# nwihardjo/SpaghettiSearch

Hardware: AMD Instinct MI355X
Metric: pagerank_iters_per_sec (higher is better)
Workload: dtype f64

## Files before the change

spaghettisearch_amd/csrc/ctx.hip:

```cpp
#include "common.hpp"
#include <chrono>

#include <unordered_map>

namespace ss {

namespace {
struct Pool {
    std::mutex mu;
    std::multimap<std::pair<int, size_t>, void*> free_blocks;
    std::unordered_map<void*, std::pair<int, size_t>> live;
    size_t held = 0, limit = (size_t)64 << 30;
    double miss_ms = 0.0;
    uint64_t misses = 0;
    int contexts = 0;
};
Pool& pool() { static Pool* p = new Pool(); return *p; }
size_t size_class(size_t b) {
    if (b <= 4096) return 4096;
    size_t p2 = 4096;
    while (p2 < b) p2 <<= 1;
    if (p2 <= ((size_t)1 << 20)) return p2;
    const size_t step = p2 >> 4;
    return (b + step - 1) / step * step;
}
}

hipError_t pool_alloc(void** out, size_t bytes) {
    Pool& P = pool();
    const size_t cls = size_class(bytes);
    int dev = 0;
    (void)hipGetDevice(&dev);
    {
        std::lock_guard<std::mutex> lk(P.mu);
        auto it = P.free_blocks.find({dev, cls});
        if (it != P.free_blocks.end()) {
            *out = it->second;
            P.free_blocks.erase(it);
            P.held -= cls;
            P.live[*out] = {dev, cls};
            return hipSuccess;
        }
    }
    const auto tm0 = std::chrono::steady_clock::now();
    hipError_t e = hipMalloc(out, cls);
    {
        std::lock_guard<std::mutex> lk(P.mu);
        P.miss_ms += std::chrono::duration<double, std::milli>(std::chrono::steady_clock::now() - tm0).count();
        P.misses++;
    }
    if (e != hipSuccess) {
        (void)hipGetLastError();
        pool_trim();
        e = hipMalloc(out, cls);
    }
    if (e == hipSuccess) {
        std::lock_guard<std::mutex> lk(P.mu);
        P.live[*out] = {dev, cls};
    }
    return e;
}

static thread_local bool t_device_idle = false;

void pool_free_batch(void* const* blocks, size_t count) {
    if (!count) return;
    {
        int cur = 0;
        (void)hipGetDevice(&cur);
        if (device_wedged(cur)) return;
    }
    (void)hipDeviceSynchronize();
    t_device_idle = true;
    for (size_t i = 0; i < count; i++) pool_free(blocks[i]);
    t_device_idle = false;
}

void pool_free(void* p) {
    if (!p) return;
    Pool& P = pool();
    size_t cls = 0, limit = 0;
    int dev = 0;
    {
        std::lock_guard<std::mutex> lk(P.mu);
        auto it = P.live.find(p);
        if (it != P.live.end()) { dev = it->second.first; cls = it->second.second; P.live.erase(it); }
        limit = P.limit;
    }
    if (device_wedged(dev)) return;
    if (cls && cls <= limit / 2) {
        int cur = 0;
        (void)hipGetDevice(&cur);
        if (cur != dev || !t_device_idle) {
            if (cur != dev) (void)hipSetDevice(dev);
            (void)hipDeviceSynchronize();
            if (cur != dev) (void)hipSetDevice(cur);
        }
        std::vector<void*> evict;
        {
            std::lock_guard<std::mutex> lk(P.mu);
            while (P.held + cls > P.limit && !P.free_blocks.empty()) {
                auto last = std::prev(P.free_blocks.end());
                if (last->first.second <= cls) break;
                evict.push_back(last->second);
                P.held -= last->first.second;
                P.free_blocks.erase(last);
            }
            if (P.held + cls <= P.limit) {
                P.free_blocks.emplace(std::make_pair(dev, cls), p);
                P.held += cls;
                p = nullptr;
            }
        }
        for (void* q : evict) (void)hipFree(q);
        if (!p) return;
    }
    (void)hipFree(p);
}

void pool_stats(uint64_t* misses, double* miss_ms) {
    std::lock_guard<std::mutex> lk(pool().mu);
    *misses = pool().misses;
    *miss_ms = pool().miss_ms;
}
void pool_context_count(int delta) {
    bool last = false;
    {
        std::lock_guard<std::mutex> lk(pool().mu);
        pool().contexts += delta;
        last = delta < 0 && pool().contexts <= 0;
    }
    if (last) pool_trim();
}

void pool_trim() {
    Pool& P = pool();
    std::multimap<std::pair<int, size_t>, void*> take;
    {
        std::lock_guard<std::mutex> lk(P.mu);
        take.swap(P.free_blocks);
        P.held = 0;
    }
    for (auto& kv : take) (void)hipFree(kv.second);
}

void pool_set_limit(size_t bytes) {
    {
        std::lock_guard<std::mutex> lk(pool().mu);
        pool().limit = bytes;
    }
    pool_trim();
}

static std::mutex g_err_mu;
static std::string g_err;
void set_global_error(const std::string& msg) {
    std::lock_guard<std::mutex> lk(g_err_mu);
    g_err = msg;
}
}

extern "C" {

int32_t ss_abi_version(void) { return SS_ABI_VERSION; }

int32_t ss_init(int32_t device_id, ss_ctx** out) {
    if (!out) {
        ss::set_global_error("ss_init: out is NULL");
        return SS_ERR_INVALID;
    }
    *out = nullptr;
    int n_dev = 0;
    hipError_t e = hipGetDeviceCount(&n_dev);
    if (e != hipSuccess || n_dev <= 0) {
        ss::set_global_error(std::string("ss_init: no HIP device (") + hipGetErrorString(e) + ")");
        return SS_ERR_NO_DEVICE;
    }
    if (device_id < 0 || device_id >= n_dev) {
        ss::set_global_error("ss_init: device_id out of range");
        return SS_ERR_INVALID;
    }
    ss_ctx* ctx = new (std::nothrow) ss_ctx();
    if (!ctx) return SS_ERR_OOM;
    ctx->device = device_id;
    if ((e = hipSetDevice(device_id)) != hipSuccess) {
        ss::set_global_error(std::string("ss_init: hipSetDevice: ") + hipGetErrorString(e));
        delete ctx;
        return SS_ERR_NO_DEVICE;
    }
    hipDeviceProp_t prop;
    if ((e = hipGetDeviceProperties(&prop, device_id)) != hipSuccess) {
        ss::set_global_error(std::string("ss_init: hipGetDeviceProperties: ") + hipGetErrorString(e));
        delete ctx;
        return SS_ERR_NO_DEVICE;
    }
    if (std::strncmp(prop.gcnArchName, "gfx950", 6) != 0) {
        ss::set_global_error(std::string("ss_init: device is ") + prop.gcnArchName +
                             ", this library is built for gfx950 (MI355X) only");
        delete ctx;
        return SS_ERR_NO_DEVICE;
    }
    ctx->cu_count = prop.multiProcessorCount;
    ctx->total_mem = prop.totalGlobalMem;
    if ((e = hipStreamCreateWithFlags(&ctx->own_stream, hipStreamNonBlocking)) != hipSuccess) {
        ss::set_global_error(std::string("ss_init: hipStreamCreate: ") + hipGetErrorString(e));
        delete ctx;
        return SS_ERR_HIP;
    }
    ctx->stream = ctx->own_stream;
    int prio_lo = 0, prio_hi = 0;
    (void)hipDeviceGetStreamPriorityRange(&prio_lo, &prio_hi);
    if ((e = hipStreamCreateWithPriority(&ctx->comm_stream, hipStreamNonBlocking, prio_hi)) != hipSuccess) {
        ss::set_global_error(std::string("ss_init: hipStreamCreate (comm): ") + hipGetErrorString(e));
        (void)hipStreamDestroy(ctx->own_stream);
        delete ctx;
        return SS_ERR_HIP;
    }
    for (int k = 0; k < 3; k++)
        for (int j = 0; j < 2; j++)
            if ((e = hipEventCreate(&ctx->ev[k][j])) != hipSuccess) {
                ss::set_global_error(std::string("ss_init: hipEventCreate: ") + hipGetErrorString(e));
                delete ctx;
                return SS_ERR_HIP;
            }
    if ((e = hipHostMalloc(reinterpret_cast<void**>(&ctx->h_pin), ss_ctx::PIN_SCRATCH, hipHostMallocDefault)) != hipSuccess) {
        ss::set_global_error(std::string("ss_init: hipHostMalloc: ") + hipGetErrorString(e));
        delete ctx;
        return SS_ERR_HIP;
    }
    ss::pool_context_count(+1);
    *out = ctx;
    return SS_OK;
}

int32_t ss_shutdown(ss_ctx* ctx) {
    if (!ctx) return SS_ERR_INVALID;
    (void)hipSetDevice(ctx->device);
    const bool stuck = !ss::try_unwedge(ctx);
    (void)ss_comm_destroy(ctx);
    if (!stuck) (void)hipStreamSynchronize(ctx->stream);
    for (int k = 0; k < 3; k++)
        for (int j = 0; j < 2; j++)
            if (ctx->ev[k][j]) (void)hipEventDestroy(ctx->ev[k][j]);
    if (ctx->comm_stream && !stuck) { (void)hipStreamSynchronize(ctx->comm_stream); (void)hipStreamDestroy(ctx->comm_stream); }
    for (hipStream_t ws : ctx->wave_stream)
        if (ws && !stuck) { (void)hipStreamSynchronize(ws); (void)hipStreamDestroy(ws); }
    if (ctx->own_stream && !stuck) (void)hipStreamDestroy(ctx->own_stream);
    if (ctx->h_pin) (void)hipHostFree(ctx->h_pin);
    for (auto& b : ctx->pin_cache) (void)hipHostFree(b.p);
    delete ctx;
    ss::pool_context_count(-1);
    return SS_OK;
}

int32_t ss_set_stream(ss_ctx* ctx, void* hip_stream) {
    if (!ctx) return SS_ERR_INVALID;
    std::lock_guard<std::recursive_mutex> lk(ctx->mu);
    SS_HIP(ctx, hipStreamSynchronize(ctx->stream));
    ctx->stream = hip_stream ? reinterpret_cast<hipStream_t>(hip_stream) : ctx->own_stream;
    return SS_OK;
}

static const char* const k_option_names[] = {
    "comm.timeout_ms",
    "pr.force_narrow",
    "pr.wire_f32",
    "pr.narrow_wave",
    "pr.t_quad",
    "pr.blocks_per_cu",
    "mem.pool_mb",
    "pr.deal_snake",
    "pr.affine_lag",
    "pr.affine",
    "pr.items_per_wave",
    "pr.persistent",
    "pr.persistent_blocks",
    "pr.n_class_order",
    "pr.class_order",
    "pr.stagger",
    "pr.deal_global",
    "pr.share_zero_rows",
    "pr.item_turns",
    "graph.late_free",
    "pr.trace",
    "score.collect_pinned",
    "score.pipeline_slices",
    "score.timing",
    "score.trace",
    "pr.probe_hot",
    "pr.topic_blocks",
    "tfidf.blocks",
    "tfidf.bucket_shift",
    "tfidf.head_min_run",
    "tfidf.bucket_min",
    "score.wave",
    "score.wave_max_terms",
    "score.wave_min_list",
    "score.wave_share_pct",
    "score.wave_slice_target",
    "score.wave_big_pct",
    "score.wave_big_x100",
    "score.small",
    "score.small_max_batch",
    "score.small_batch",
    "score.small_cap",
    "score.pipeline",
    "score.grade_slices",
    "score.wave_small_x100",
    "score.exact_all",
    "score.slice_target",
    "score.separate_merge",
    "passage.lds_events",
    "lexicon.chunk_terms",
};

int32_t ss_set_option(ss_ctx* ctx, const char* name, int64_t value) {
    if (!ctx || !name) return SS_ERR_INVALID;
    std::lock_guard<std::recursive_mutex> lk(ctx->mu);
    for (const char* n : k_option_names)
        if (std::strcmp(n, name) == 0) {
            if (value == SS_OPTION_DEFAULT) ctx->options.erase(name);
            else ctx->options[name] = value;
            if (std::strcmp(name, "mem.pool_mb") == 0) ss::pool_set_limit(value == SS_OPTION_DEFAULT ? (size_t)64 << 30 : (size_t)std::max<int64_t>(0, value) << 20);
            return SS_OK;
        }
    return ctx->fail(SS_ERR_INVALID, "ss_set_option: unknown option '%s'", name);
}

int32_t ss_synchronize(ss_ctx* ctx) {
    if (!ctx) return SS_ERR_INVALID;
    std::lock_guard<std::recursive_mutex> lk(ctx->mu);
    SS_HIP(ctx, hipSetDevice(ctx->device));
    SS_TRY(ss::sync_bounded(ctx, ctx->stream, "ss_synchronize"));
    return SS_OK;
}

const char* ss_last_error(ss_ctx* ctx) {
    if (ctx) return ctx->last_error.c_str();
    static thread_local std::string tl;
    {
        std::lock_guard<std::mutex> lk(ss::g_err_mu);
        tl = ss::g_err;
    }
    return tl.c_str();
}

int32_t ss_last_kernel_ms(ss_ctx* ctx, int32_t kind, float* ms_out) {
    if (!ctx || !ms_out || kind < 0 || kind > 2) return SS_ERR_INVALID;
    std::lock_guard<std::recursive_mutex> lk(ctx->mu);
    if (!ctx->ev_valid[kind]) return ctx->fail(SS_ERR_STATE, "ss_last_kernel_ms: no timed call of kind %d yet", kind);
    SS_HIP(ctx, hipEventSynchronize(ctx->ev[kind][1]));
    SS_HIP(ctx, hipEventElapsedTime(ms_out, ctx->ev[kind][0], ctx->ev[kind][1]));
    return SS_OK;
}

}
```

spaghettisearch_amd/csrc/pagerank.hip:

```cpp
#include "pr_device.hpp"

#include <algorithm>
#include <chrono>
#include <cmath>
#include <memory>

namespace {

__global__ void k_pr_item_ranges(WorkItem* __restrict__ work, uint32_t n_items, const uint32_t* __restrict__ in_ptr) {
    const uint32_t i = blockIdx.x * blockDim.x + threadIdx.x;
    if (i >= n_items) return;
    WorkItem w = work[i];
    switch (w.kind) {
        case V_ROWW: w.beg = in_ptr[w.row]; w.end = in_ptr[w.row + 1]; break;
        case V_SEG:
            w.beg = in_ptr[w.row] + w.count * SEGW;
            w.end = min(in_ptr[w.row + 1], w.beg + SEGW);
            break;
        case V_QUAD:
        case V_DEG: w.beg = in_ptr[w.row]; w.end = in_ptr[w.row + w.count]; break;
        default: return;
    }
    work[i] = w;
}

__global__ __launch_bounds__(TPB) void k_pr_remap_src(const uint32_t* __restrict__ in_src, uint32_t* __restrict__ out, size_t n_edges, uint32_t pos_nd,
                                                      uint32_t cnt_nd, const uint32_t* __restrict__ outdeg, const uint32_t* __restrict__ sh_deg,
                                                      uint32_t n_shared, uint32_t zrow) {
    for (size_t e = (size_t)blockIdx.x * TPB + threadIdx.x; e < n_edges; e += (size_t)gridDim.x * TPB) {
        uint32_t w = NT_LOAD(&in_src[e]);
        const uint32_t s = w & SRC_MASK;
        if (s >= pos_nd) {
            uint32_t row = zrow;
            if (s < cnt_nd && n_shared) {
                const uint32_t od = outdeg[s];
                uint32_t lo = 0, hi = n_shared;
                while (lo < hi) {
                    const uint32_t mid = (lo + hi) >> 1;
                    if (sh_deg[mid] < od) lo = mid + 1; else hi = mid;
                }
                if (lo < n_shared && sh_deg[lo] == od) row = zrow + 1 + lo;
            }
            w = (w & ~SRC_MASK) | row;
        }
        NT_STORE(w, &out[e]);
    }
}

template <int GW>
__global__ __launch_bounds__(TPB) void k_pr_begin(PrParams p) {
    const int lane = threadIdx.x & 63;
    const int t = lane % GW;
    const double x0 = p.x0[t];
    double* __restrict__ Tw = p.tab_wr[1];
    double csum = 0.0;
    for (uint32_t i = blockIdx.x * TPB + threadIdx.x; i < p.n_shared * (uint32_t)GW; i += gridDim.x * TPB)
        Tw[(size_t)(p.zrow + 1) * GW + i] = p.d * x0 / (double)p.sh_deg[i / GW];
    const size_t n_el = ((size_t)p.sl_nd + p.sl_d) * GW;
    for (size_t i = (size_t)blockIdx.x * TPB + threadIdx.x; i < n_el; i += (size_t)gridDim.x * TPB) {
        const uint32_t lrow = (uint32_t)(i / GW);
        const bool real = lrow < p.sl_nd ? lrow < p.cnt_nd : (lrow - p.sl_nd) < p.cnt_d;
        p.x[i] = real ? x0 : 0.0;
        if (lrow < p.sl_nd) {
            double c = 0.0;
            if (real) c = p.d * x0 / (double)p.outdeg[lrow];
            if ((p.world == 1 || lrow + 2 < p.sl_nd) && lrow < p.tab_rows) Tw[i] = c;
            csum += c;
        }
    }
    block_reduce_and_publish<GW>(p, 0.0, csum, Tw, true);
}

template <int GW>
__global__ void k_pr_finalize(PrParams p, const double* __restrict__ table, int is_begin) {
    if (threadIdx.x != 0 || blockIdx.x != 0) return;
    if (!is_begin && p.ctl->n_active == 0) return;
    double dl[MAXK], cs[MAXK];
    for (int k = 0; k < MAXK; k++) { dl[k] = 0.0; cs[k] = 0.0; }
    for (int r = 0; r < p.world; r++) {
        const size_t base = ((size_t)r * p.sl_nd + (p.sl_nd - 2)) * GW;
        for (int k = 0; k < GW; k++) {
            cs[k] += table[base + k];
            dl[k] += table[base + GW + k];
        }
    }
    finalize_ctl(p, dl, cs, is_begin != 0);
}

template <int GW>
__global__ void k_pr_read(const double* __restrict__ x, const PrCtl* __restrict__ ctl, const uint32_t* __restrict__ old_id,
                          uint32_t sl_nd, uint32_t cnt_nd, uint32_t pos_nd, uint32_t sl_d, uint32_t cnt_d, uint32_t pos_d,
                          uint64_t id0_nd, uint64_t id0_d, int k_topics, uint64_t out_stride,
                          int by_original_id, uint32_t* __restrict__ ids_out, double* __restrict__ out,
                          const uint32_t* __restrict__ memb, uint32_t ts_mask) {
    const size_t n_rows = (size_t)cnt_nd + cnt_d;
    size_t i = (size_t)blockIdx.x * blockDim.x + threadIdx.x;
    if (i >= n_rows) return;
    const uint32_t lrow = i < cnt_nd ? (uint32_t)i : sl_nd + (uint32_t)(i - cnt_nd);
    const uint64_t iid = lrow < sl_nd ? id0_nd + lrow : id0_d + (lrow - sl_nd);
    const uint32_t orig = old_id[iid];
    const size_t o = by_original_id ? (size_t)orig : i;
    if (ids_out) ids_out[i] = orig;
    const bool zero = lrow < sl_nd ? lrow >= pos_nd : (lrow - sl_nd) >= pos_d;
    const uint32_t mb = memb ? memb[lrow] & ts_mask : 0u;
    for (int k = 0; k < k_topics; k++)
        out[(size_t)k * out_stride + o] = zero ? (((mb >> k) & 1u) ? ctl->xz_in[k] : ctl->xz[k]) : x[(size_t)lrow * GW + k];
}

__global__ void k_pr_memb(const uint64_t* __restrict__ set_ptr, const uint32_t* __restrict__ set_nodes, int k_topics, uint64_t n_nodes,
                          const uint32_t* __restrict__ new_id, uint64_t nd_int, uint32_t sl_nd, uint32_t sl_d, int rank,
                          uint32_t* __restrict__ memb, uint32_t* __restrict__ seen, uint32_t* __restrict__ err) {
    const uint64_t total = set_ptr[k_topics];
    for (uint64_t i = (uint64_t)blockIdx.x * blockDim.x + threadIdx.x; i < total; i += (uint64_t)gridDim.x * blockDim.x) {
        int k = 0;
        while (k + 1 < k_topics && set_ptr[k + 1] <= i) k++;
        const uint32_t v = set_nodes[i];
        if ((uint64_t)v >= n_nodes) { atomicOr(err, 1u); continue; }
        if (atomicOr(&seen[v], 1u << k) & (1u << k)) { atomicOr(err, 2u); continue; }
        const uint64_t iid = new_id[v];
        uint32_t lrow;
        int owner;
        if (iid < nd_int) { owner = (int)(iid / sl_nd); lrow = (uint32_t)(iid % sl_nd); }
        else { owner = (int)((iid - nd_int) / sl_d); lrow = sl_nd + (uint32_t)((iid - nd_int) % sl_d); }
        if (owner == rank) atomicOr(&memb[lrow], 1u << k);
    }
}
__global__ void k_pr_memb_zero_count(const uint32_t* __restrict__ memb, uint32_t sl_nd, uint32_t cnt_nd, uint32_t pos_nd, uint32_t cnt_d,
                                     uint32_t pos_d, int k_topics, unsigned long long* __restrict__ cnt) {
    const uint32_t z_nd = cnt_nd - pos_nd, n_zero = z_nd + (cnt_d - pos_d);
    for (uint32_t i = blockIdx.x * blockDim.x + threadIdx.x; i < n_zero; i += gridDim.x * blockDim.x) {
        const uint32_t lrow = i < z_nd ? pos_nd + i : sl_nd + pos_d + (i - z_nd);
        const uint32_t mb = memb[lrow];
        for (int k = 0; k < k_topics; k++)
            if ((mb >> k) & 1u) atomicAdd(&cnt[k], 1ull);
    }
}

template <int GW, int POL>
__global__ __launch_bounds__(TPB) void k_pr_probe(const double* __restrict__ T, const uint32_t* __restrict__ in_src, size_t n_edges,
                                                  uint32_t n_rows, int mode, double* __restrict__ sink, uint32_t hot) {
    if constexpr (GW >= 8) {
        constexpr int NSLOT = 64 / GW;
        const int lane = threadIdx.x & 63, wave = threadIdx.x >> 6;
        const int t = lane % GW, slot = lane / GW, gbase = lane - t;
        const size_t groups = (size_t)gridDim.x * WAVES * NSLOT;
        const size_t gi = ((size_t)blockIdx.x * WAVES + wave) * NSLOT + slot;
        const size_t n_chunks = n_edges / CH;
        const size_t per = (n_chunks + groups - 1) / groups;
        size_t c = min(gi * per, n_chunks);
        const size_t c_hi = min(c + per, n_chunks);
        double acc = 0.0;
        for (; c < c_hi; c++) {
            constexpr int R = CH / GW;
            uint32_t src[R];
#pragma unroll
            for (int r = 0; r < R; r++) {
                const size_t e = c * CH + (size_t)(r * GW + t);
                uint32_t v = NT_LOAD(&in_src[e]) & SRC_MASK;
                if (mode == 1) v = (uint32_t)(((uint64_t)(v * 2654435761u + (uint32_t)e * 40503u) * n_rows) >> 32);
                if (mode == 2) v = (uint32_t)(e % n_rows);
                src[r] = v;
            }
            double v[CH];
#pragma unroll
            for (int j = 0; j < CH; j++) {
                const uint32_t sj = (uint32_t)__shfl((int)src[j / GW], gbase + (j % GW), 64);
                const double* a = &T[(size_t)sj * GW + t];
                if constexpr (POL == 0) v[j] = *a;
                else if constexpr (POL == 1) v[j] = __builtin_nontemporal_load(a);
                else if constexpr (POL == 2) v[j] = __hip_atomic_load(a, __ATOMIC_RELAXED, __HIP_MEMORY_SCOPE_AGENT);
                else if constexpr (POL == 3) v[j] = sj < hot ? *a : __builtin_nontemporal_load(a);
                else v[j] = sj < hot ? *a : __hip_atomic_load(a, __ATOMIC_RELAXED, __HIP_MEMORY_SCOPE_AGENT);
            }
#pragma unroll
            for (int j = 0; j < CH; j++) acc += v[j];
        }
        sink[((size_t)blockIdx.x * TPB + threadIdx.x)] = acc;
    }
}

}

namespace {

void pick_kernel(const ss_ctx* ctx, ss_pr* pr, int k, uint64_t table_rows) {
    const bool force_narrow = ctx->opt("pr.force_narrow", 0) != 0, narrow_wave = ctx->opt("pr.narrow_wave", 1) != 0;
    if (k > 2) {
        pr->kernel = PR_SWEEP;
        pr->gw = k <= 8 ? 8 : 16;
    } else if (force_narrow) {
        pr->kernel = PR_STEP;
        pr->gw = k;
    } else if (narrow_wave) {
        pr->kernel = PR_SWEEP_N;
        pr->gw = k;
    } else if (table_rows * 64 <= (64ull << 20)) {
        pr->kernel = PR_SWEEP;
        pr->gw = 8;
    } else {
        pr->kernel = PR_STEP;
        pr->gw = k;
    }
    pr->nwave = pr->kernel == PR_SWEEP_N;
    const int64_t want = ctx->opt("pr.persistent", 0);
    pr->persist_mode = want == 2 ? 2 : 1;
    pr->persist = pr->nwave && pr->g->world == 1 && !ctx->opt("pr.affine", 0) && want > 0;
}

template <int GW>
void launch_begin(ss_pr* pr, hipStream_t st, unsigned nb) {
    hipLaunchKernelGGL(k_pr_begin<GW>, dim3(nb), dim3(TPB), 0, st, pr->prm);
}
template <int GW>
void launch_finalize(ss_pr* pr, hipStream_t st, int is_begin) {
    hipLaunchKernelGGL(k_pr_finalize<GW>, dim3(1), dim3(64), 0, st, pr->prm, (const double*)pr->tab0.p, is_begin);
}
template <int GW>
__global__ __launch_bounds__(TPB) void k_pr_read_orig(const double* __restrict__ x, const PrCtl* __restrict__ ctl, const uint32_t* __restrict__ new_id,
                                                      uint64_t n, uint32_t sl_nd, uint32_t pos_nd, uint32_t pos_d, int k_topics,
                                                      double* __restrict__ out, const uint32_t* __restrict__ memb, uint32_t ts_mask) {
    const uint64_t v = (uint64_t)blockIdx.x * blockDim.x + threadIdx.x;
    if (v >= n) return;
    const uint32_t lrow = new_id[v];
    const bool zero = lrow < sl_nd ? lrow >= pos_nd : (lrow - sl_nd) >= pos_d;
    double r[GW];
    if (!zero) {
        if constexpr (GW >= 2) {
            const double2* const row = reinterpret_cast<const double2*>(x + (size_t)lrow * GW);
#pragma unroll
            for (int j = 0; j < GW / 2; j++) { const double2 t = row[j]; r[2 * j] = t.x; r[2 * j + 1] = t.y; }
        } else {
            r[0] = x[lrow];
        }
    } else {
        const uint32_t mb = memb ? memb[lrow] & ts_mask : 0u;
#pragma unroll
        for (int k = 0; k < GW; k++) r[k] = ((mb >> k) & 1u) ? ctl->xz_in[k] : ctl->xz[k];
    }
#pragma unroll
    for (int k = 0; k < GW; k++)
        if (k < k_topics) out[(size_t)k * n + v] = r[k];
}

template <int GW>
void launch_read(ss_pr* pr, hipStream_t st, int by_orig, uint64_t stride, uint32_t* ids, double* out) {
    const ss_graph* g = pr->g;
    const size_t n_rows = (size_t)g->cnt_nd + g->cnt_d;
    if (!n_rows) return;
    if (by_orig && g->world == 1 && !ids && stride == g->n) {
        hipLaunchKernelGGL(k_pr_read_orig<GW>, dim3(ss::div_up(g->n, TPB)), dim3(TPB), 0, st, (const double*)pr->x.p, (const PrCtl*)pr->ctl.p,
                           (const uint32_t*)g->new_id.p, g->n, g->sl_nd, pr->prm.pos_nd, pr->prm.pos_d, pr->k, out, pr->prm.memb, pr->prm.ts_mask);
        return;
    }
    hipLaunchKernelGGL(k_pr_read<GW>, dim3(ss::div_up(n_rows, TPB)), dim3(TPB), 0, st, (const double*)pr->x.p,
                       (const PrCtl*)pr->ctl.p, (const uint32_t*)g->old_id.p, g->sl_nd, g->cnt_nd, pr->prm.pos_nd, g->sl_d, g->cnt_d,
                       pr->prm.pos_d,
                       (uint64_t)g->rank * g->sl_nd, g->nd_int + (uint64_t)g->rank * g->sl_d, pr->k, stride, by_orig, ids, out,
                       pr->prm.memb, pr->prm.ts_mask);
}

#define SS_GW_DISPATCH(gw, fn, ...)          \
    switch (gw) {                            \
        case 1: fn<1>(__VA_ARGS__); break;   \
        case 2: fn<2>(__VA_ARGS__); break;   \
        case 8: fn<8>(__VA_ARGS__); break;   \
        default: fn<16>(__VA_ARGS__); break; \
    }

}

namespace ss {
unsigned begin_blocks(const ss_pr* pr) { return std::max(1u, std::min(2048u, ss::div_up((size_t)pr->g->n_local() * pr->gw, TPB))); }
void pr_launch_begin(ss_pr* pr, hipStream_t st, unsigned nb) { SS_GW_DISPATCH(pr->gw, launch_begin, pr, st, nb); }
void pr_launch_step(ss_pr* pr, hipStream_t st) {
    switch (pr->kernel) {
        case PR_STEP: pr_step_launch(pr, st); break;
        case PR_SWEEP: pr_sweep_launch(pr, st); break;
        case PR_SWEEP_N: pr_sweep_n_launch(pr, st); break;
    }
}
void pr_launch_finalize(ss_pr* pr, hipStream_t st, int is_begin) { SS_GW_DISPATCH(pr->gw, launch_finalize, pr, st, is_begin); }
}

namespace {

PlanOptions plan_options(const ss_ctx* ctx, const ss_pr* pr, size_t n_local) {
    const bool small = n_local <= ((size_t)4 << 20);
    PlanOptions o;
    o.t_quad = (uint32_t)ctx->opt("pr.t_quad", pr->nwave ? 256 : 128);
    o.item_turns = (uint32_t)std::max<int64_t>(1, std::min<int64_t>(64, ctx->opt("pr.item_turns", pr->nwave ? (small ? 1 : 4) : (small ? 4 : 8))));
    o.items_per_wave = pr->nwave ? (size_t)std::max<int64_t>(1, ctx->opt("pr.items_per_wave", 4)) : 1;
    o.deal_snake = ctx->opt("pr.deal_snake", PlanOptions::AUTO);
    o.deal_global = ctx->opt("pr.deal_global", pr->nwave && pr->gw == 1 ? 1 : 2);
    o.blocks_per_cu = ctx->opt("pr.blocks_per_cu", PlanOptions::AUTO);
    o.class_order = ctx->opt("pr.class_order", 235401);
    o.n_class_order = ctx->opt("pr.n_class_order", small ? 2310 : 123);
    o.stagger = ctx->opt("pr.stagger", 0);
    return o;
}

constexpr int OCC_MULTI_N = 3;
int blocks_per_cu(int row, int gw) {
    static std::mutex occ_mu;
    static int occ_cache[4][MAXK + 1] = {};
    std::lock_guard<std::mutex> lk_occ(occ_mu);
    int& occ = occ_cache[row][gw];
    if (!occ) {
        int per_cu = 0;
        switch (row) {
            case PR_STEP: per_cu = ss::pr_step_occupancy(gw); break;
            case PR_SWEEP: per_cu = ss::pr_sweep_occupancy(gw); break;
            case PR_SWEEP_N: per_cu = ss::pr_sweep_n_occupancy(gw); break;
            default: per_cu = ss::pr_multi_n_occupancy(gw); break;
        }
        occ = std::max(per_cu, 1);
    }
    return occ;
}
unsigned grid_for(const ss_ctx* ctx, const ss_pr* pr, const PlanOptions& opt, int per_cu, size_t n_items) {
    per_cu = (int)std::max<int64_t>(1, opt.blocks_per_cu == PlanOptions::AUTO ? per_cu : opt.blocks_per_cu);
    if (pr->persist) {
        const int admit = std::max(1, blocks_per_cu(OCC_MULTI_N, pr->gw) - 2);
        per_cu = (int)std::max<int64_t>(1, std::min<int64_t>(std::min(admit, std::max(1, per_cu / 2)), ctx->opt("pr.persistent_blocks", 4)));
    }
    return pr->kernel != PR_STEP ? (unsigned)std::min<size_t>(std::max<size_t>(1, ss::div_up(n_items, (size_t)WAVES * opt.items_per_wave)), (size_t)ctx->cu_count * per_cu)
                                 : (unsigned)std::min<size_t>(n_items, (size_t)ctx->cu_count * 8);
}

void fill_params(ss_pr* pr, const Cut& cut, const PlanOptions& opt, double damping, double eps, int32_t max_iter, int32_t k_topics) {
    const ss_graph* g = pr->g;
    PrParams& p = pr->prm;
    p.in_ptr = g->in_ptr.p;
    p.in_src = g->in_src.p;
    p.outdeg = g->outdeg.p;
    p.x = pr->x.p;
    if (g->world == 1) {
        p.tab_rd[0] = pr->tab0.p; p.tab_wr[0] = pr->tab1.p;
        p.tab_rd[1] = pr->tab1.p; p.tab_wr[1] = pr->tab0.p;
    } else {
        p.tab_rd[0] = p.tab_rd[1] = pr->tab0.p;
        p.tab_wr[0] = p.tab_wr[1] = pr->send.p;
    }
    p.work = pr->work.p;
    p.partials = pr->partials.p;
    p.segpart = pr->segpart.p;
    p.rowticket = pr->rowticket.p;
    p.ctl = pr->ctl.p;
    p.x0 = pr->x0.p;
    p.d = damping;
    p.teleport = 1.0 - damping;
    p.eps = eps;
    p.tele_n = p.teleport * (double)g->n;
    p.max_iter = max_iter;
    p.k_topics = k_topics;
    p.world = g->world;
    p.sl_nd = g->sl_nd;
    p.cnt_nd = g->cnt_nd;
    p.sl_d = g->sl_d;
    p.cnt_d = g->cnt_d;
    p.seg_edges = cut.seg_edges;
    p.n_items = (uint32_t)cut.items.size();
    p.pos_nd = cut.pos_nd;
    p.pos_d = cut.pos_d;
    p.zrow = (uint32_t)g->nd_int;
    p.tab_rows = g->sl_nd;
    p.woff = pr->woff.p;
    p.stagger_div = opt.stagger != 0 ? (uint32_t)std::max(g->ctx->cu_count, 1) : 0u;
    p.stagger_code = opt.stagger >= 10 ? (uint32_t)(opt.stagger - 10) : 0u;
    p.class_order = pack_class_order(opt.class_order);
    p.n_order = pack_n_order(opt.n_class_order);
}

uint64_t fnv1a(const void* q, size_t n, uint64_t h = 0xcbf29ce484222325ull) {
    const unsigned char* b = static_cast<const unsigned char*>(q);
    for (size_t i = 0; i < n; i++) { h ^= b[i]; h *= 0x100000001b3ull; }
    return h;
}
void trace_plan(const ss_pr* pr, const std::vector<WorkItem>& work, const std::vector<uint32_t>& woff) {
    const PrParams& p = pr->prm;
    const double sd[] = {p.d, p.teleport, p.eps, p.tele_n};
    const uint32_t su[] = {(uint32_t)p.max_iter, (uint32_t)p.k_topics, (uint32_t)p.world, p.sl_nd, p.cnt_nd, p.sl_d, p.cnt_d, p.seg_edges, p.n_items,
                           p.pos_nd, p.pos_d, p.ts_mask, p.zrow, p.stagger_div, p.stagger_code, p.class_order, p.n_order};
    fprintf(stderr, "[pr trace] plan: work %016llx (%zu items)  woff %016llx  params %016llx  nblocks %u\n",
            (unsigned long long)fnv1a(work.data(), work.size() * sizeof(WorkItem)), work.size(),
            (unsigned long long)fnv1a(woff.data(), woff.size() * sizeof(uint32_t)),
            (unsigned long long)fnv1a(su, sizeof(su), fnv1a(sd, sizeof(sd))), pr->nblocks);
}

int32_t alloc_tables(ss_pr* pr, hipStream_t st, size_t rows) {
    const ss_graph* g = pr->g;
    ss_ctx* ctx = g->ctx;
    const size_t GW = (size_t)pr->gw;
    SS_HIP(ctx, pr->tab0.alloc(rows * GW));
    SS_HIP(ctx, hipMemsetAsync(pr->tab0.p, 0, std::max<size_t>(pr->tab0.bytes(), 8), st));
    if (g->world == 1) {
        SS_HIP(ctx, pr->tab1.alloc(rows * GW));
        SS_HIP(ctx, hipMemsetAsync(pr->tab1.p, 0, std::max<size_t>(pr->tab1.bytes(), 8), st));
    } else {
        SS_HIP(ctx, pr->send.alloc((size_t)g->sl_nd * GW));
        SS_HIP(ctx, hipMemsetAsync(pr->send.p, 0, std::max<size_t>(pr->send.bytes(), 8), st));
    }
    return SS_OK;
}
int32_t unshare_rows(ss_pr* pr, hipStream_t st) {
    if (!pr->prm.share) return SS_OK;
    const ss_graph* g = pr->g;
    SS_HIP(g->ctx, hipStreamSynchronize(st));
    SS_TRY(alloc_tables(pr, st, (size_t)g->nd_int + 1));
    pr->src_shared.release();
    pr->sh_deg.release();
    PrParams& p = pr->prm;
    p.tab_rd[0] = pr->tab0.p; p.tab_wr[0] = pr->tab1.p;
    p.tab_rd[1] = pr->tab1.p; p.tab_wr[1] = pr->tab0.p;
    p.in_src = g->in_src.p;
    p.sh_deg = nullptr;
    p.n_shared = 0;
    p.share = 0;
    p.zrow = (uint32_t)g->nd_int;
    p.tab_rows = g->sl_nd;
    return SS_OK;
}

#ifdef SS_PR_WAVETIME
void dump_wave_loads(const Cut& cut, const std::vector<double>& cost, const std::vector<uint32_t>& owner, uint32_t nw) {
    FILE* f = open_dump("pr_load.csv");
    if (!f) return;
    std::vector<double> wl(nw, 0.0), wcls((size_t)nw * 6, 0.0);
    for (size_t i = 0; i < cut.items.size(); i++) {
        int kc = 0; while (kc < 5 && i >= cut.vbeg[kc + 1]) kc++;
        wl[owner[i]] += cost[i]; wcls[(size_t)owner[i] * 6 + kc] += cost[i];
    }
    fprintf(f, "wave,load,c0,c1,c2,c3,c4,c5\n");
    for (uint32_t w = 0; w < nw; w++) fprintf(f, "%u,%.2f,%.2f,%.2f,%.2f,%.2f,%.2f,%.2f\n", w, wl[w], wcls[(size_t)w * 6], wcls[(size_t)w * 6 + 1], wcls[(size_t)w * 6 + 2], wcls[(size_t)w * 6 + 3], wcls[(size_t)w * 6 + 4], wcls[(size_t)w * 6 + 5]);
    fclose(f);
}
#endif

}

extern "C" {

int32_t ss_pr_create(ss_graph* g, double damping, double eps, int32_t max_iter, int32_t k_topics,
                     const int32_t* n_topic, ss_pr** out) {
    if (!g) return SS_ERR_INVALID;
    ss_ctx* ctx = g->ctx;
    std::lock_guard<std::recursive_mutex> lk(ctx->mu);
    if (!out) return ctx->fail(SS_ERR_INVALID, "ss_pr_create: out is NULL");
    *out = nullptr;
    if (k_topics < 1 || !n_topic) return ctx->fail(SS_ERR_INVALID, "ss_pr_create: k_topics < 1 or n_topic NULL");
    if (k_topics > MAXK) return ctx->fail(SS_ERR_UNSUPPORTED, "ss_pr_create: k_topics %d > %d per state (ss_pagerank_run splits larger K)", k_topics, MAXK);
    SS_HIP(ctx, hipSetDevice(ctx->device));
    hipStream_t st = ctx->stream;

    ss_pr* pr = new (std::nothrow) ss_pr();
    if (!pr) return ctx->fail(SS_ERR_OOM, "ss_pr_create: host OOM");
    std::unique_ptr<ss_pr> guard(pr);
    pr->g = g;
    pr->k = k_topics;
    pick_kernel(ctx, pr, k_topics, g->nd_int);
    const int GW = pr->gw;
    const bool vitems = pr->kernel != PR_STEP;
    const int GI = pr->nwave ? 8 : GW;
    const size_t n_local = g->n_local();
    if (((uint64_t)g->nd_int + 1) * GW * 8 >= (1ull << 32))
        return ctx->fail(SS_ERR_UNSUPPORTED, "ss_pr_create: contribution table of %llu rows x %d topics exceeds 4 GiB (shard the graph over more ranks)",
                         (unsigned long long)g->nd_int, GW);

    const bool trace = ctx->opt("pr.trace", 0) != 0;
    auto t_now = [] { return std::chrono::steady_clock::now(); };
    auto t_ms = [](std::chrono::steady_clock::time_point a, std::chrono::steady_clock::time_point b) { return std::chrono::duration<double, std::milli>(b - a).count(); };
    SS_HIP(ctx, pr->x.alloc(n_local * GW));
    bool share = GW >= 8 && g->world == 1 && ctx->opt("pr.affine", 0) == 0 && ctx->opt("pr.share_zero_rows", 1) != 0;
    if (!share) SS_TRY(alloc_tables(pr, st, (size_t)g->nd_int + 1));

    const auto tc0 = t_now();
    const PlanOptions opt = plan_options(ctx, pr, n_local);
    Cut cut = cut_items(g->h_indeg_nd, g->h_indeg_d, g->sl_nd, GI, pr->nwave, opt);
    const uint32_t n_tail = g->cnt_nd - cut.pos_nd;
    struct PinGuard { ss_ctx* c; void* p = nullptr; size_t cap = 0; ~PinGuard() { c->pin_free(p, cap); } } tail_od{ctx};
    if (share && n_tail == 0) {
        share = false;
        SS_TRY(alloc_tables(pr, st, (size_t)g->nd_int + 1));
    }
    if (share) {
        tail_od.p = ctx->pin_alloc((size_t)n_tail * sizeof(uint32_t), &tail_od.cap);
        if (!tail_od.p) return ctx->fail(SS_ERR_OOM, "ss_pr_create: no pinned host memory for %u out-degrees", n_tail);
        SS_HIP(ctx, hipMemcpyAsync(tail_od.p, g->outdeg.p + cut.pos_nd, (size_t)n_tail * sizeof(uint32_t), hipMemcpyDeviceToHost, st));
    }
    const auto tc1 = t_now();
    const int per_cu = blocks_per_cu(pr->kernel, GW);
    const auto tc1a = t_now();
    pr->nblocks = grid_for(ctx, pr, opt, per_cu, cut.items.size());
    static const std::vector<uint32_t> no_woff;
    const std::vector<uint32_t>* woff = &no_woff;
    if (vitems) {
        const uint32_t nw = pr->nblocks * WAVES;
        const auto td0 = t_now();
        const std::vector<double>& cost = item_costs(cut, g->h_indeg_nd, g->h_indeg_d, g->sl_nd, GI, pr->nwave);
        const auto td0a = t_now();
        std::vector<uint32_t>& owner = deal_items(cut, cost, nw, pr->nwave, opt);
#ifdef SS_PR_WAVETIME
        dump_wave_loads(cut, cost, owner, nw);
#endif
        const auto td1 = t_now();
        if (trace) fprintf(stderr, "[pr trace]   deal: occupancy query %.2f ms, costs %.3f ms, owners %.3f ms\n", t_ms(tc1, tc1a), t_ms(td0, td0a), t_ms(td0a, td1));
        woff = &place_items(cut, owner, nw);
        if (trace) fprintf(stderr, "[pr trace]   deal: placement %.3f ms\n", t_ms(td1, t_now()));
    }
    const std::vector<WorkItem>& items = cut.items;

    g->settle();
    const auto tc2 = t_now();
    SharedRows sh;
    if (share) {
        SS_HIP(ctx, hipStreamSynchronize(st));
        const auto ts0 = t_now();
        sh = plan_shared_rows(static_cast<const uint32_t*>(tail_od.p), n_tail, cut.pos_nd);
        const auto ts1 = t_now();
        SS_TRY(alloc_tables(pr, st, (size_t)sh.table_rows));
        SS_HIP(ctx, pr->sh_deg.alloc(sh.deg.size()));
        SS_HIP(ctx, hipMemcpyAsync(pr->sh_deg.p, sh.deg.data(), sh.deg.size() * sizeof(uint32_t), hipMemcpyHostToDevice, st));
        SS_HIP(ctx, pr->src_shared.alloc(g->e_local));
        if (g->e_local)
            hipLaunchKernelGGL(k_pr_remap_src, dim3((unsigned)std::min<uint64_t>(ss::div_up(g->e_local, TPB), (uint64_t)ctx->cu_count * 16)), dim3(TPB), 0, st,
                               (const uint32_t*)g->in_src.p, pr->src_shared.p, (size_t)g->e_local, cut.pos_nd, g->cnt_nd, (const uint32_t*)g->outdeg.p,
                               (const uint32_t*)pr->sh_deg.p, (uint32_t)sh.deg.size(), sh.zrow);
        if (trace) fprintf(stderr, "[pr trace]   shared rows: %u rows without in-edges -> %zu shared rows (host %.3f ms), table %llu rows\n", n_tail, sh.deg.size(),
                           t_ms(ts0, ts1), (unsigned long long)sh.table_rows);
    }
    SS_HIP(ctx, pr->partials.alloc(((size_t)std::max(pr->nblocks, ss::begin_blocks(pr)) + 8) * 2 * GW));
    SS_HIP(ctx, pr->segpart.alloc((size_t)std::max(cut.nsegs, 1u) * GW));
    SS_HIP(ctx, pr->rowticket.alloc(std::max(cut.nmulti, 1u)));
    SS_HIP(ctx, hipMemsetAsync(pr->rowticket.p, 0, pr->rowticket.bytes(), st));
    SS_HIP(ctx, pr->woff.alloc(std::max<size_t>(woff->size(), 8)));
    if (!woff->empty()) SS_HIP(ctx, hipMemcpyAsync(pr->woff.p, woff->data(), woff->size() * sizeof(uint32_t), hipMemcpyHostToDevice, st));
    SS_HIP(ctx, pr->work.alloc(items.size()));
    SS_HIP(ctx, hipMemcpyAsync(pr->work.p, items.data(), items.size() * sizeof(WorkItem), hipMemcpyHostToDevice, st));
    if (vitems)
        hipLaunchKernelGGL(k_pr_item_ranges, dim3(ss::div_up(items.size(), TPB)), dim3(TPB), 0, st, pr->work.p, (uint32_t)items.size(), (const uint32_t*)g->in_ptr.p);
    SS_HIP(ctx, pr->ctl.alloc(1));
    SS_HIP(ctx, hipMemsetAsync(pr->ctl.p, 0, sizeof(PrCtl), st));
    double h_x0[MAXK];
    for (int k = 0; k < MAXK; k++) h_x0[k] = k < k_topics ? 1.0 / (double)n_topic[k] : 0.0;
    SS_HIP(ctx, pr->x0.alloc(MAXK));
    SS_HIP(ctx, hipMemcpyAsync(pr->x0.p, h_x0, sizeof(h_x0), hipMemcpyHostToDevice, st));
    SS_HIP(ctx, hipStreamSynchronize(st));
    if (trace) fprintf(stderr, "[pr trace] ss_pr_create: build_work %.2f ms (%zu items), edge ranges + deal %.2f ms, alloc + upload %.2f ms\n", t_ms(tc0, tc1), items.size(), t_ms(tc1, tc2), t_ms(tc2, t_now()));
    if (trace) fprintf(stderr, "[pr trace] where the state lives: x %p  tab0 %p  tab1 %p  in_src %p  in_ptr %p  outdeg %p  work %p  woff %p\n", (void*)pr->x.p, (void*)pr->tab0.p,
                       (void*)pr->tab1.p, (void*)g->in_src.p, (void*)g->in_ptr.p, (void*)g->outdeg.p, (void*)pr->work.p, (void*)pr->woff.p);

    fill_params(pr, cut, opt, damping, eps, max_iter, k_topics);
    if (share) {
        PrParams& p = pr->prm;
        p.in_src = pr->src_shared.p;
        p.sh_deg = pr->sh_deg.p;
        p.n_shared = (uint32_t)sh.deg.size();
        p.share = 1;
        p.zrow = sh.zrow;
        p.tab_rows = cut.pos_nd;
    }
    if (trace) trace_plan(pr, items, *woff);
    g->users++;
    *out = guard.release();
    return SS_OK;
}

int32_t ss_pr_set_teleport(ss_pr* pr, const uint64_t* set_ptr, const uint32_t* set_nodes) {
    if (!pr) return SS_ERR_INVALID;
    ss_ctx* ctx = pr->g->ctx;
    std::lock_guard<std::recursive_mutex> lk(ctx->mu);
    SS_HIP(ctx, hipSetDevice(ctx->device));
    if (pr->begun) return ctx->fail(SS_ERR_STATE, "ss_pr_set_teleport: call before ss_pr_begin");
    hipStream_t st = ctx->stream;
    PrParams& p = pr->prm;
    if (!set_ptr) {
        p.memb = nullptr; p.tin = nullptr; p.nz_in = nullptr; p.ts_mask = 0;
        return SS_OK;
    }
    const ss_graph* g = pr->g;
    const int K = pr->k;
    SS_TRY(unshare_rows(pr, st));
    std::vector<uint64_t> h_ptr(K + 1);
    SS_HIP(ctx, ss::copy_in(ctx->stream, h_ptr.data(), set_ptr, (K + 1) * sizeof(uint64_t)));
    if (h_ptr[0] != 0) return ctx->fail(SS_ERR_INVALID, "ss_pr_set_teleport: set_ptr[0] != 0");
    for (int k = 0; k < K; k++)
        if (h_ptr[k + 1] < h_ptr[k]) return ctx->fail(SS_ERR_INVALID, "ss_pr_set_teleport: set_ptr not non-decreasing");
    const uint64_t total = h_ptr[K];
    if (total && !set_nodes) return ctx->fail(SS_ERR_INVALID, "ss_pr_set_teleport: set_nodes is NULL");
    double h_tin[MAXK];
    uint32_t mask = 0;
    for (int k = 0; k < MAXK; k++) {
        h_tin[k] = 0.0;
        if (k < K && h_ptr[k + 1] > h_ptr[k]) {
            mask |= 1u << k;
            h_tin[k] = p.teleport * (double)g->n / (double)(h_ptr[k + 1] - h_ptr[k]);
        }
    }
    const size_t n_local = g->n_local();
    ss::DevBuf<uint64_t> d_ptr;
    ss::DevBuf<uint32_t> d_nodes, d_err, d_seen;
    ss::DevBuf<unsigned long long> d_cnt;
    SS_HIP(ctx, d_ptr.alloc(K + 1));
    SS_HIP(ctx, d_seen.alloc(g->n));
    SS_HIP(ctx, hipMemsetAsync(d_seen.p, 0, std::max<size_t>(d_seen.bytes(), 4), st));
    SS_HIP(ctx, d_nodes.alloc(total));
    SS_HIP(ctx, d_err.alloc(1));
    SS_HIP(ctx, d_cnt.alloc(MAXK));
    SS_HIP(ctx, pr->memb.alloc(n_local));
    SS_HIP(ctx, pr->tin.alloc(MAXK));
    SS_HIP(ctx, pr->nz_in.alloc(MAXK));
    SS_HIP(ctx, hipMemcpyAsync(d_ptr.p, h_ptr.data(), (K + 1) * sizeof(uint64_t), hipMemcpyHostToDevice, st));
    if (total) SS_HIP(ctx, hipMemcpyAsync(d_nodes.p, set_nodes, total * sizeof(uint32_t), hipMemcpyDefault, st));
    SS_HIP(ctx, hipMemsetAsync(pr->memb.p, 0, std::max<size_t>(pr->memb.bytes(), 4), st));
    SS_HIP(ctx, hipMemsetAsync(d_err.p, 0, sizeof(uint32_t), st));
    SS_HIP(ctx, hipMemsetAsync(d_cnt.p, 0, MAXK * sizeof(unsigned long long), st));
    if (total)
        hipLaunchKernelGGL(k_pr_memb, dim3(std::min<unsigned>(ss::div_up(total, TPB), 4096u)), dim3(TPB), 0, st, (const uint64_t*)d_ptr.p,
                           (const uint32_t*)d_nodes.p, K, g->n, (const uint32_t*)g->new_id.p, g->nd_int, std::max(g->sl_nd, 1u), std::max(g->sl_d, 1u),
                           g->rank, pr->memb.p, d_seen.p, d_err.p);
    const uint32_t n_zero = (g->cnt_nd - p.pos_nd) + (g->cnt_d - p.pos_d);
    if (n_zero)
        hipLaunchKernelGGL(k_pr_memb_zero_count, dim3(std::min<unsigned>(ss::div_up(n_zero, TPB), 4096u)), dim3(TPB), 0, st,
                           (const uint32_t*)pr->memb.p, g->sl_nd, g->cnt_nd, p.pos_nd, g->cnt_d, p.pos_d, K, d_cnt.p);
    SS_HIP(ctx, hipGetLastError());
    uint32_t h_err = 0;
    unsigned long long h_cnt[MAXK];
    SS_HIP(ctx, ss::fetch(ctx, st, &h_err, d_err.p, sizeof(h_err), h_cnt, d_cnt.p, sizeof(h_cnt)));
    if (h_err & 1u) return ctx->fail(SS_ERR_INVALID, "ss_pr_set_teleport: a teleport set holds a node id >= n_nodes");
    if (h_err & 2u) return ctx->fail(SS_ERR_INVALID, "ss_pr_set_teleport: a teleport set lists a node twice (the ids of a set must be distinct)");
    double h_nz[MAXK];
    for (int k = 0; k < MAXK; k++) h_nz[k] = (double)h_cnt[k];
    SS_HIP(ctx, hipMemcpyAsync(pr->tin.p, h_tin, sizeof(h_tin), hipMemcpyHostToDevice, st));
    SS_HIP(ctx, hipMemcpyAsync(pr->nz_in.p, h_nz, sizeof(h_nz), hipMemcpyHostToDevice, st));
    SS_HIP(ctx, hipStreamSynchronize(st));
    p.memb = pr->memb.p;
    p.tin = pr->tin.p;
    p.nz_in = pr->nz_in.p;
    p.ts_mask = mask;
    return SS_OK;
}

int32_t ss_pr_destroy(ss_pr* pr) {
#ifdef SS_PR_WAVETIME
    if (pr) ss::pr_dump_wave_times(pr);
#endif

    if (!pr) return SS_ERR_INVALID;
    ss_ctx* ctx = pr->g->ctx;
    std::lock_guard<std::recursive_mutex> lk(ctx->mu);
    (void)hipSetDevice(ctx->device);
    if (!ss::device_wedged(ctx->device)) {
        (void)hipStreamSynchronize(ctx->stream);
        (void)hipStreamSynchronize(ctx->comm_stream);
    }
    pr->g->users--;
    delete pr;
    return SS_OK;
}

int32_t ss_pr_begin(ss_pr* pr) {
    if (!pr) return SS_ERR_INVALID;
    ss_ctx* ctx = pr->g->ctx;
    std::lock_guard<std::recursive_mutex> lk(ctx->mu);
    SS_HIP(ctx, hipSetDevice(ctx->device));
    if (pr->need_finalize) return ctx->fail(SS_ERR_STATE, "ss_pr_begin: pending exchange/finalize");
    SS_HIP(ctx, hipMemsetAsync(&pr->ctl.p->ticket, 0, sizeof(uint32_t), ctx->stream));
    ss::pr_launch_begin(pr, ctx->stream, ss::begin_blocks(pr));
    SS_HIP(ctx, hipGetLastError());
    pr->begun = true;
    if (pr->g->world > 1) {
        pr->need_finalize = true;
        pr->finalize_is_begin = true;
    }
    return SS_OK;
}

int32_t ss_pr_step(ss_pr* pr, int32_t n_steps) {
    if (!pr) return SS_ERR_INVALID;
    ss_ctx* ctx = pr->g->ctx;
    std::lock_guard<std::recursive_mutex> lk(ctx->mu);
    SS_HIP(ctx, hipSetDevice(ctx->device));
    if (!pr->begun) return ctx->fail(SS_ERR_STATE, "ss_pr_step: ss_pr_begin not called");
    if (pr->need_finalize) return ctx->fail(SS_ERR_STATE, "ss_pr_step: pending exchange/finalize");
    if (n_steps < 1) return ctx->fail(SS_ERR_INVALID, "ss_pr_step: n_steps < 1");
    if (pr->g->world > 1 && n_steps != 1) return ctx->fail(SS_ERR_INVALID, "ss_pr_step: world>1 needs an exchange after every step");
    SS_HIP(ctx, hipEventRecord(ctx->ev[0][0], ctx->stream));
    if (pr->persist && !pr->prm.memb && !pr->prm.aff) {
        ss::pr_multi_n_launch(pr, ctx->stream, (int)n_steps);
    } else {
        for (int i = 0; i < n_steps; i++) ss::pr_launch_step(pr, ctx->stream);
    }
    SS_HIP(ctx, hipEventRecord(ctx->ev[0][1], ctx->stream));
    ctx->ev_valid[0] = true;
    SS_HIP(ctx, hipGetLastError());
    if (pr->g->world > 1) {
        pr->need_finalize = true;
        pr->finalize_is_begin = false;
    }
    return SS_OK;
}

int32_t ss_pr_finalize(ss_pr* pr) {
    if (!pr) return SS_ERR_INVALID;
    ss_ctx* ctx = pr->g->ctx;
    std::lock_guard<std::recursive_mutex> lk(ctx->mu);
    SS_HIP(ctx, hipSetDevice(ctx->device));
    if (pr->g->world == 1) return ctx->fail(SS_ERR_STATE, "ss_pr_finalize: world==1 folds the finalize into the sweep");
    if (!pr->need_finalize) return ctx->fail(SS_ERR_STATE, "ss_pr_finalize: nothing to finalize");
    ss::pr_launch_finalize(pr, ctx->stream, pr->finalize_is_begin ? 1 : 0);
    SS_HIP(ctx, hipGetLastError());
    pr->need_finalize = false;
    return SS_OK;
}

int32_t ss_pr_exchange_buffers(ss_pr* pr, void** send_dev, uint64_t* send_bytes, void** recv_dev, uint64_t* recv_bytes) {
    if (!pr) return SS_ERR_INVALID;
    ss_ctx* ctx = pr->g->ctx;
    if (pr->g->world == 1) return ctx->fail(SS_ERR_STATE, "ss_pr_exchange_buffers: world==1 has no exchange");
    if (send_dev) *send_dev = pr->send.p;
    if (send_bytes) *send_bytes = pr->send.bytes();
    if (recv_dev) *recv_dev = pr->tab0.p;
    if (recv_bytes) *recv_bytes = (uint64_t)pr->g->nd_int * pr->gw * sizeof(double);
    return SS_OK;
}

int32_t ss_pr_exchange(ss_pr* pr, int32_t allreduce) {
    if (!pr) return SS_ERR_INVALID;
    ss_ctx* ctx = pr->g->ctx;
    std::lock_guard<std::recursive_mutex> lk(ctx->mu);
    SS_HIP(ctx, hipSetDevice(ctx->device));
    const ss_graph* g = pr->g;
    if (g->world == 1) return ctx->fail(SS_ERR_STATE, "ss_pr_exchange: world==1 has no exchange");
    if (!pr->need_finalize) return ctx->fail(SS_ERR_STATE, "ss_pr_exchange: nothing to exchange (call after ss_pr_begin / ss_pr_step)");
    if (!ctx->comm || ctx->comm_world != g->world || ctx->comm_rank != g->rank)
        return ctx->fail(SS_ERR_STATE, "ss_pr_exchange: the context's communicator (rank %d of %d) does not match the graph's shard (rank %d of %d)",
                         ctx->comm ? ctx->comm_rank : -1, ctx->comm ? ctx->comm_world : 0, g->rank, g->world);
    const size_t slice = (size_t)g->sl_nd * pr->gw;
    if (!allreduce && ctx->opt("pr.wire_f32", 0) != 0) {
        SS_HIP(ctx, ss::pr_wire_alloc(pr));
        ss::pr_wire_pack(pr, ctx->stream);
        SS_TRY(ss::comm_allgather(ctx, pr->wire_send.p, pr->wire_recv.p, ss::pr_wire_floats(pr) * sizeof(float)));
        ss::pr_wire_unpack(pr, ctx->stream);
        return SS_OK;
    }
    if (!allreduce) return ss::comm_allgather(ctx, pr->send.p, pr->tab0.p, slice * sizeof(double));
    SS_HIP(ctx, hipMemsetAsync(pr->tab0.p, 0, pr->tab0.bytes(), ctx->stream));
    SS_HIP(ctx, hipMemcpyAsync(pr->tab0.p + (size_t)g->rank * slice, pr->send.p, slice * sizeof(double), hipMemcpyDeviceToDevice, ctx->stream));
    return ss::comm_allreduce_f64(ctx, pr->tab0.p, pr->tab0.p, slice * (size_t)g->world);
}

int32_t ss_pr_status(ss_pr* pr, int32_t* iters_out, int32_t* n_active, int32_t* sweeps, double* last_delta_out,
                     double* last_total_out) {
    if (!pr) return SS_ERR_INVALID;
    ss_ctx* ctx = pr->g->ctx;
    std::lock_guard<std::recursive_mutex> lk(ctx->mu);
    SS_HIP(ctx, hipSetDevice(ctx->device));
    const PrCtl* hp = nullptr;
    SS_TRY(read_ctl(ctx, pr, ctx->stream, "ss_pr_status", &hp));
    const PrCtl h = *hp;
    if (h.stuck) return ctx->fail(SS_ERR_STATE, "ss_pr_status: the multi-sweep kernel gave up waiting between two sweeps (its grid of %u blocks was not resident: "
                                  "other kernels held the CUs for seconds); the state is void — set option pr.persistent = 0 and run again", pr->nblocks);
    for (int k = 0; k < pr->k; k++) {
        if (iters_out) iters_out[k] = h.iters[k];
        if (last_delta_out) last_delta_out[k] = h.delta[k];
        if (last_total_out) last_total_out[k] = h.S[k];
    }
    if (n_active) *n_active = h.n_active;
    if (sweeps) *sweeps = h.sweep;
    return SS_OK;
}

int32_t ss_pr_read_local(ss_pr* pr, uint32_t* ids_out, double* rank_out) {
    if (!pr || !rank_out) return SS_ERR_INVALID;
    ss_ctx* ctx = pr->g->ctx;
    std::lock_guard<std::recursive_mutex> lk(ctx->mu);
    SS_HIP(ctx, hipSetDevice(ctx->device));
    const ss_graph* g = pr->g;
    const size_t n_rows = (size_t)g->cnt_nd + g->cnt_d;
    ss::DevBuf<uint32_t> d_ids;
    ss::DevBuf<double> d_out;
    SS_HIP(ctx, d_ids.alloc(n_rows));
    SS_HIP(ctx, d_out.alloc(n_rows * pr->k));
    SS_GW_DISPATCH(pr->gw, launch_read, pr, ctx->stream, 0, (uint64_t)n_rows, d_ids.p, d_out.p);
    SS_HIP(ctx, hipGetLastError());
    if (ids_out && n_rows) SS_HIP(ctx, hipMemcpyAsync(ids_out, d_ids.p, n_rows * sizeof(uint32_t), hipMemcpyDefault, ctx->stream));
    if (n_rows) SS_HIP(ctx, hipMemcpyAsync(rank_out, d_out.p, n_rows * pr->k * sizeof(double), hipMemcpyDefault, ctx->stream));
    SS_HIP(ctx, hipStreamSynchronize(ctx->stream));
    return SS_OK;
}

int32_t ss_pr_read(ss_pr* pr, double* rank_out) {
    if (!pr || !rank_out) return SS_ERR_INVALID;
    ss_ctx* ctx = pr->g->ctx;
    std::lock_guard<std::recursive_mutex> lk(ctx->mu);
    SS_HIP(ctx, hipSetDevice(ctx->device));
    const ss_graph* g = pr->g;
    if (g->world != 1) return ctx->fail(SS_ERR_STATE, "ss_pr_read: world>1, use ss_pr_read_local");
    hipPointerAttribute_t pa{};
    const bool dev_out = hipPointerGetAttributes(&pa, rank_out) == hipSuccess && pa.type == hipMemoryTypeDevice;
    (void)hipGetLastError();
    ss::DevBuf<double> d_out;
    if (!dev_out) SS_HIP(ctx, d_out.alloc((size_t)g->n * pr->k));
    SS_GW_DISPATCH(pr->gw, launch_read, pr, ctx->stream, 1, (uint64_t)g->n, (uint32_t*)nullptr, dev_out ? rank_out : d_out.p);
    SS_HIP(ctx, hipGetLastError());
    if (!dev_out) SS_HIP(ctx, hipMemcpyAsync(rank_out, d_out.p, (size_t)g->n * pr->k * sizeof(double), hipMemcpyDefault, ctx->stream));
    SS_HIP(ctx, hipStreamSynchronize(ctx->stream));
    return SS_OK;
}

int32_t ss_pr_probe(ss_pr* pr, int32_t mode, int32_t n_reps, float* ms_out) {
    if (!pr || !ms_out) return SS_ERR_INVALID;
    ss_ctx* ctx = pr->g->ctx;
    std::lock_guard<std::recursive_mutex> lk(ctx->mu);
    SS_HIP(ctx, hipSetDevice(ctx->device));
    if (pr->gw < 8) return ctx->fail(SS_ERR_UNSUPPORTED, "ss_pr_probe: the probe mirrors the chunked gather of the K >= 5 kernels");
    if (mode < 0 || (mode & 7) > 2 || (mode >> 3) > 4 || n_reps < 1) return ctx->fail(SS_ERR_INVALID, "ss_pr_probe: mode 0..2 (+ 8 * gather cache policy 0..4), n_reps >= 1");
    const int pol = mode >> 3;
    mode &= 7;
    const uint32_t hot = (uint32_t)ctx->opt("pr.probe_hot", 24576);
    const ss_graph* g = pr->g;
    const unsigned nb = (unsigned)ctx->cu_count * 8;
    ss::DevBuf<double> sink;
    SS_HIP(ctx, sink.alloc((size_t)nb * TPB));
    hipEvent_t e0, e1;
    SS_HIP(ctx, hipEventCreate(&e0));
    SS_HIP(ctx, hipEventCreate(&e1));
    hipStream_t st = ctx->stream;
    ss::DevBuf<double> full;
    if (pr->prm.share) {
        SS_HIP(ctx, full.alloc(((size_t)g->nd_int + 1) * pr->gw));
        SS_HIP(ctx, hipMemsetAsync(full.p, 0, full.bytes(), ctx->stream));
    }
    const double* T = pr->prm.share ? full.p : pr->tab0.p;
    for (int r = 0; r < n_reps + 1; r++) {
        if (r == 1) SS_HIP(ctx, hipEventRecord(e0, st));
#define SS_PROBE_LAUNCH(GWV, POLV) hipLaunchKernelGGL((k_pr_probe<GWV, POLV>), dim3(nb), dim3(TPB), 0, st, T, (const uint32_t*)g->in_src.p, (size_t)g->e_local, (uint32_t)g->nd_int, mode, sink.p, hot)
        if (pr->gw == 8) SS_PROBE_LAUNCH(8, 0);
        else switch (pol) {
            case 0: SS_PROBE_LAUNCH(16, 0); break;
            case 1: SS_PROBE_LAUNCH(16, 1); break;
            case 2: SS_PROBE_LAUNCH(16, 2); break;
            case 3: SS_PROBE_LAUNCH(16, 3); break;
            default: SS_PROBE_LAUNCH(16, 4); break;
        }
    }
    SS_HIP(ctx, hipEventRecord(e1, st));
    SS_HIP(ctx, hipEventSynchronize(e1));
    float ms = 0.f;
    SS_HIP(ctx, hipEventElapsedTime(&ms, e0, e1));
    (void)hipEventDestroy(e0);
    (void)hipEventDestroy(e1);
    SS_HIP(ctx, hipGetLastError());
    *ms_out = ms / (float)n_reps;
    return SS_OK;
}

}
```

spaghettisearch_amd/csrc/pr_plan.hpp:

```cpp
#pragma once
#include "sorted_degrees.hpp"

#include <algorithm>
#include <cstdint>
#include <utility>
#include <vector>

namespace {

constexpr int TPB = 256;
constexpr int WAVES = TPB / 64;
constexpr int CH = 16;
constexpr uint32_t SEGW = 2048;

enum : uint32_t { W_SEG = 0, W_WAVE = 1, W_GROUP = 2, W_ZERO = 3,
                  V_SEG = 8,
                  V_ROWW = 9,
                  V_QUAD = 10,
                  V_DEG = 11,
                  V_ZERO = 12 };

struct WorkItem {
    uint32_t kind;
    uint32_t row;
    uint32_t count;
    uint32_t nseg;
    uint32_t sbase;
    uint32_t tix;
    uint32_t beg, end;
};

constexpr uint32_t plan_div_up(uint64_t a, uint64_t b) { return (uint32_t)((a + b - 1) / b); }

struct PlanOptions {
    static constexpr int64_t AUTO = INT64_MIN;
    uint32_t t_quad = 128;
    uint32_t item_turns = 4;
    size_t items_per_wave = 1;
    int64_t deal_snake = AUTO;
    int64_t deal_global = 2;
    int64_t blocks_per_cu = AUTO;
    int64_t class_order = 235401;
    int64_t n_class_order = 2310;
    int64_t stagger = 0;
};

struct PlanScratch {
    std::vector<WorkItem> seg, rwg, wav, grp, zer;
    std::vector<WorkItem> vseg, vroww, vquad, vdeg[3], vzero;
    std::vector<WorkItem> items, dealt;
    std::vector<double> cost, load;
    std::vector<uint32_t> owner, by_load, idx, order, bucket, woff, cnt;
    std::vector<std::pair<double, uint32_t>> key;
};
inline PlanScratch& plan_scratch() {
    static thread_local PlanScratch s;
    return s;
}

struct Cut {
    std::vector<WorkItem>& items;
    uint32_t nsegs = 0, nmulti = 0;
    uint32_t seg_edges = 0;
    uint32_t pos_nd = 0, pos_d = 0;
    uint32_t vbeg[7] = {0};
};

inline Cut cut_items(const ss::SortedDegrees& nd, const ss::SortedDegrees& d, uint32_t sl_nd, int gw, bool lane_rows, const PlanOptions& opt) {
    PlanScratch& s = plan_scratch();
    Cut cut{s.items};
    uint32_t& nsegs = cut.nsegs;
    uint32_t& nmulti = cut.nmulti;
    const uint32_t NSLOT = 64 / gw;
    const uint32_t T_SEG = 32 * NSLOT;
    const uint32_t T_WAVE = 2 * NSLOT;
    const uint32_t seg_edges = cut.seg_edges = 128 * NSLOT;
    auto &seg = s.seg, &rwg = s.rwg, &wav = s.wav, &grp = s.grp, &zer = s.zer;
    auto &vseg = s.vseg, &vroww = s.vroww, &vquad = s.vquad, &vzero = s.vzero;
    auto& vdeg = s.vdeg;
    for (auto* v : {&seg, &rwg, &wav, &grp, &zer, &vseg, &vroww, &vquad, &vdeg[0], &vdeg[1], &vdeg[2], &vzero}) v->clear();
    auto emit_v = [&](const ss::SortedDegrees& deg, uint32_t row0, bool non_dangling, uint32_t& n_pos) {
        const uint32_t cnt = (uint32_t)deg.size();
        const uint32_t T_MULTI = 4096, T_DEG = 8;
        const uint32_t T_QUAD = opt.t_quad;
        const uint32_t item_turns = opt.item_turns;
        size_t j_at = 0, j_lim = 0;
        const size_t n_run = deg.val.size();
        auto deg_at = [&](uint32_t r) -> uint32_t {
            while (deg.start[j_at + 1] <= r) j_at++;
            return deg.val[j_at];
        };
        auto end_above = [&](uint32_t lim) -> uint32_t {
            while (j_lim < n_run && deg.val[j_lim] > lim) j_lim++;
            return deg.start[j_lim];
        };
        uint32_t r = 0;
        for (; r < cnt && deg_at(r) > T_MULTI; r++) {
            const uint32_t ns = (deg_at(r) + SEGW - 1) / SEGW;
            const uint32_t tix = nmulti++;
            for (uint32_t sg = 0; sg < ns; sg++) vseg.push_back({V_SEG, row0 + r, sg, ns, nsegs, tix});
            nsegs += ns;
        }
        {
            const uint32_t end = std::min(cnt, end_above(T_QUAD));
            for (; r < end; r++) vroww.push_back({V_ROWW, row0 + r, 0, 0, 0, 0});
        }
        while (r < cnt && deg_at(r) > T_DEG) {
            const uint32_t nch = (deg_at(r) + CH - 1) / CH;
            const uint32_t max_groups = std::min<uint32_t>((uint32_t)gw, std::max<uint32_t>(1u, 2u * item_turns / nch));
            const uint32_t lim = std::max<uint32_t>(T_DEG, (nch - 1) * CH);
            const uint32_t end = end_above(lim);
            const uint32_t same = end > r ? end - r : 0u;
            const uint32_t rows = std::min<uint32_t>(same, max_groups * NSLOT);
            vquad.push_back({V_QUAD, row0 + r, rows, nch, 0, 0});
            r += rows;
        }
        while (r < cnt && deg_at(r) > 0) {
            const uint32_t D = deg_at(r);
            const uint32_t run = deg.start[j_at + 1] - r;
            const uint32_t R = D <= 2 ? 8 : D <= 4 ? 4 : 2;
            const uint32_t per_item = lane_rows ? 64u * item_turns : NSLOT * R * item_turns;
            auto& out = vdeg[R == 2 ? 0 : R == 4 ? 1 : 2];
            for (uint32_t o = 0; o < run; o += per_item) out.push_back({V_DEG, row0 + r + o, std::min(per_item, run - o), D, 0, 0});
            r += run;
        }
        n_pos = r;
        const uint32_t ZERO_ROWS = 16 * NSLOT;
        if (non_dangling)
            for (uint32_t o = r; o < cnt; o += ZERO_ROWS) vzero.push_back({V_ZERO, row0 + o, std::min<uint32_t>(ZERO_ROWS, cnt - o), 0, 0, 0});
    };
    auto emit = [&](const ss::SortedDegrees& deg, uint32_t row0, bool non_dangling, uint32_t& n_pos) {
        if (gw >= 8) { emit_v(deg, row0, non_dangling, n_pos); return; }
        const uint32_t cnt = (uint32_t)deg.size();
        const uint32_t a = deg.first_at_most(T_SEG);
        const uint32_t c = std::max(a, deg.first_at_most(0));
        for (uint32_t r = 0; r < a; r++) {
            const uint32_t ns = (deg[r] + seg_edges - 1) / seg_edges;
            const uint32_t tix = ns > 1 ? nmulti++ : 0;
            for (uint32_t sg = 0; sg < ns; sg++) seg.push_back({W_SEG, row0 + r, sg, ns, nsegs, tix});
            nsegs += ns;
        }
        {
            const uint32_t b = std::min(c, std::max(a, deg.first_at_most(T_WAVE)));
            for (uint32_t r = a; r < b; r += WAVES) wav.push_back({W_WAVE, row0 + r, std::min<uint32_t>(WAVES, b - r), 0, 0, 0});
            const uint32_t GROUP_ROWS = WAVES * NSLOT * 4;
            for (uint32_t r = b; r < c; r += GROUP_ROWS) grp.push_back({W_GROUP, row0 + r, std::min<uint32_t>(GROUP_ROWS, c - r), 0, 0, 0});
        }
        n_pos = c;
        const uint32_t ZERO_ROWS = (TPB * 8) / gw;
        if (non_dangling)
            for (uint32_t r = c; r < cnt; r += ZERO_ROWS) zer.push_back({W_ZERO, row0 + r, std::min<uint32_t>(ZERO_ROWS, cnt - r), 0, 0, 0});
    };
    emit(nd, 0, true, cut.pos_nd);
    const size_t vquad_split = vquad.size();
    emit(d, sl_nd, false, cut.pos_d);
    auto& items = cut.items;
    auto& vbeg = cut.vbeg;
    items.clear();
    items.reserve(seg.size() + rwg.size() + wav.size() + grp.size() + zer.size());
    items.insert(items.end(), seg.begin(), seg.end());
    items.insert(items.end(), rwg.begin(), rwg.end());
    items.insert(items.end(), wav.begin(), wav.end());
    items.insert(items.end(), grp.begin(), grp.end());
    items.insert(items.end(), zer.begin(), zer.end());
    vbeg[0] = (uint32_t)items.size();
    items.insert(items.end(), vseg.begin(), vseg.end());
    items.insert(items.end(), vroww.begin(), vroww.end());
    vbeg[1] = (uint32_t)items.size();
    std::inplace_merge(vquad.begin(), vquad.begin() + (ptrdiff_t)vquad_split, vquad.end(),
                       [](const WorkItem& a, const WorkItem& b) { return a.nseg > b.nseg; });
    items.insert(items.end(), vquad.begin(), vquad.end());
    for (int k = 0; k < 3; k++) {
        vbeg[2 + k] = (uint32_t)items.size();
        items.insert(items.end(), vdeg[k].begin(), vdeg[k].end());
    }
    vbeg[5] = (uint32_t)items.size();
    items.insert(items.end(), vzero.begin(), vzero.end());
    vbeg[6] = (uint32_t)items.size();
    if (items.empty()) items.push_back({W_ZERO, 0, 0, 0, 0, 0});
    return cut;
}

inline const std::vector<double>& item_costs(const Cut& cut, const ss::SortedDegrees& nd, const ss::SortedDegrees& d, uint32_t sl_nd, int gw, bool lane_rows) {
    const std::vector<WorkItem>& items = cut.items;
    std::vector<double>& cost = plan_scratch().cost;
    const uint32_t NS = 64 / gw;
    struct DegCursor {
        const ss::SortedDegrees* d;
        size_t j = 0;
        uint32_t at(uint32_t r) {
            if (r >= d->size()) return 0u;
            if (d->start[j] > r) j = d->run_of(r);
            while (d->start[j + 1] <= r) j++;
            return d->val[j];
        }
    } cur_nd{&nd}, cur_d{&d};
    auto deg_of = [&](uint32_t lrow) -> uint32_t { return lrow < sl_nd ? cur_nd.at(lrow) : cur_d.at(lrow - sl_nd); };
    cost.assign(items.size(), 0.0);
    for (size_t i = 0; i < items.size(); i++) {
        const WorkItem& w = items[i];
        double turns = 1.0;
        switch (w.kind) {
            case V_ROWW: turns = plan_div_up(deg_of(w.row), NS * CH); break;
            case V_SEG: turns = plan_div_up(std::min<uint32_t>(SEGW, deg_of(w.row) - w.count * SEGW), NS * CH) + 2.0; break;
            case V_QUAD: turns = (double)plan_div_up(w.count, NS) * w.nseg; break;
            case V_DEG: {
                if (lane_rows) { turns = (double)plan_div_up(w.count, 64u) * (0.6 + 0.2 * (w.nseg <= 2 ? 2 : w.nseg <= 4 ? 4 : 8)); break; }
                const uint32_t R = w.nseg <= 2 ? 8 : w.nseg <= 4 ? 4 : 2;
                turns = (double)plan_div_up(w.count, NS * R) * (R == 8 ? 2.5 : R == 4 ? 1.7 : 1.3);
                break;
            }
            default: turns = 0.5; break;
        }
        cost[i] = turns + 1.0;
    }
    return cost;
}

inline std::vector<uint32_t>& deal_items(const Cut& cut, const std::vector<double>& cost, uint32_t nw, bool lane_rows, const PlanOptions& opt) {
    PlanScratch& s = plan_scratch();
    const size_t n_items = cut.items.size();
    auto &owner = s.owner, &by_load = s.by_load, &idx = s.idx, &order = s.order, &bucket = s.bucket;
    auto& load = s.load;
    auto& key = s.key;
    owner.assign(n_items, 0u);
    load.assign(nw, 0.0);
    by_load.resize(nw);
    for (uint32_t w = 0; w < nw; w++) by_load[w] = w;
    const bool snake = (opt.deal_snake == PlanOptions::AUTO ? (n_items >= (size_t)8 * nw || lane_rows ? 1 : 0) : opt.deal_snake) != 0;
    const int64_t deal_mode = opt.deal_global;
    const bool global_order = deal_mode != 0;
    if (global_order) {
        constexpr uint32_t NB = 1u << 14;
        const auto bkey = [&](size_t i) { return NB - 1 - (uint32_t)std::min<double>(cost[i] * 16.0, (double)(NB - 1)); };
        bucket.assign(NB + 1, 0u);
        order.resize(n_items);
        size_t c0 = 0;
        for (int kcls = 0; kcls < (deal_mode == 2 ? 6 : 1); kcls++) {
            const size_t c1 = deal_mode == 2 ? (kcls < 5 ? std::min<size_t>(cut.vbeg[kcls + 1], n_items) : n_items) : n_items;
            if (kcls) std::fill(bucket.begin(), bucket.end(), 0u);
            for (size_t i = c0; i < c1; i++) bucket[bkey(i) + 1]++;
            for (uint32_t b = 0; b < NB; b++) bucket[b + 1] += bucket[b];
            for (size_t i = c0; i < c1; i++) order[c0 + bucket[bkey(i)]++] = (uint32_t)i;
            c0 = c1;
        }
    }
    for (size_t i0 = 0; i0 < n_items; i0 += nw) {
        const size_t n_chunk = std::min<size_t>(nw, n_items - i0);
        if (i0 && snake) {
            std::reverse(by_load.begin(), by_load.end());
        } else if (i0) {
            key.resize(nw);
            for (uint32_t w = 0; w < nw; w++) key[w] = {load[w], w};
            std::sort(key.begin(), key.end());
            for (uint32_t w = 0; w < nw; w++) by_load[w] = key[w].second;
        }
        idx.resize(n_chunk);
        for (size_t j = 0; j < n_chunk; j++) idx[j] = global_order ? order[i0 + j] : (uint32_t)(i0 + j);
        const auto falling = [&](uint32_t a, uint32_t b) { return cost[a] > cost[b]; };
        size_t run_end = 0, n_merge = 0;
        for (size_t j = 1; j <= n_chunk && !global_order; j++) {
            if (j < n_chunk && !(cost[i0 + j] > cost[i0 + j - 1])) continue;
            if (run_end) {
                if (++n_merge > 8) { std::stable_sort(idx.begin(), idx.end(), falling); break; }
                std::inplace_merge(idx.begin(), idx.begin() + (ptrdiff_t)run_end, idx.begin() + (ptrdiff_t)j, falling);
            }
            run_end = j;
        }
        for (size_t j = 0; j < n_chunk; j++) {
            owner[idx[j]] = by_load[j];
            load[by_load[j]] += cost[idx[j]];
        }
    }
    return owner;
}

inline const std::vector<uint32_t>& place_items(Cut& cut, std::vector<uint32_t>& owner, uint32_t nw) {
    PlanScratch& s = plan_scratch();
    auto& items = cut.items;
    auto &woff = s.woff, &cnt = s.cnt;
    woff.assign((size_t)nw * 8, 0);
    cnt.assign((size_t)nw * 8, 0);
    for (int k = 0; k < 6; k++) {
        const size_t i1 = k < 5 ? std::min<size_t>(cut.vbeg[k + 1], items.size()) : items.size();
        for (size_t i = std::min<size_t>(cut.vbeg[k], i1); i < i1; i++) { owner[i] = owner[i] * 8 + (uint32_t)k; cnt[owner[i]]++; }
    }
    uint32_t run_off = 0;
    for (uint32_t w = 0; w < nw; w++) {
        for (int k = 0; k < 8; k++) {
            woff[(size_t)w * 8 + k] = run_off;
            run_off += cnt[(size_t)w * 8 + k];
            cnt[(size_t)w * 8 + k] = woff[(size_t)w * 8 + k];
        }
    }
    s.dealt.resize(items.size());
    for (size_t i = 0; i < items.size(); i++) s.dealt[cnt[owner[i]]++] = items[i];
    s.dealt.push_back({V_ZERO, 0, 0, 0, 0, 0, 0, 0});
    s.dealt.push_back({V_ZERO, 0, 0, 0, 0, 0, 0, 0});
    items.swap(s.dealt);
    return woff;
}

inline uint32_t pack_class_order(int64_t code) {
    uint32_t packed = 0, seen = 0;
    for (int pos = 5; pos >= 0; pos--) {
        const uint32_t c = (uint32_t)(code % 10);
        code /= 10;
        packed |= (c & 7u) << (3 * pos);
        if (c < 6) seen |= 1u << c;
    }
    return seen == 0x3Fu ? packed : (0u | 1u << 3 | 2u << 6 | 3u << 9 | 4u << 12 | 5u << 15);
}
inline uint32_t pack_n_order(int64_t code) {
    uint32_t packed = 0, seen = 0;
    for (int pos = 3; pos >= 0; pos--) {
        const uint32_t c = (uint32_t)(code % 10);
        code /= 10;
        packed |= (c & 3u) << (2 * pos);
        if (c < 4) seen |= 1u << c;
    }
    return seen == 0xFu ? packed : (0u | 1u << 2 | 2u << 4 | 3u << 6);
}

struct SharedRows {
    std::vector<uint32_t> deg;
    uint32_t zrow = 0;
    uint32_t base = 0;
    uint64_t table_rows = 0;
    uint32_t row_of(uint32_t od) const {
        const auto it = std::lower_bound(deg.begin(), deg.end(), od);
        return it != deg.end() && *it == od ? base + (uint32_t)(it - deg.begin()) : zrow;
    }
};
inline SharedRows plan_shared_rows(const uint32_t* od, size_t n, uint32_t pos_nd) {
    SharedRows sh;
    uint32_t hi = 0;
    for (size_t i = 0; i < n; i++) hi = std::max(hi, od[i]);
    if (n && (uint64_t)hi <= 4 * (uint64_t)n + 65536) {
        std::vector<unsigned char> seen((size_t)hi + 1, 0);
        for (size_t i = 0; i < n; i++) seen[od[i]] = 1;
        for (size_t v = 0; v <= hi; v++)
            if (seen[v]) sh.deg.push_back((uint32_t)v);
    } else if (n) {
        sh.deg.assign(od, od + n);
        std::sort(sh.deg.begin(), sh.deg.end());
        sh.deg.erase(std::unique(sh.deg.begin(), sh.deg.end()), sh.deg.end());
    }
    sh.zrow = pos_nd;
    sh.base = pos_nd + 1;
    sh.table_rows = (uint64_t)pos_nd + 1 + sh.deg.size();
    return sh;
}

}
```

spaghettisearch_amd/csrc/pr_state.hpp:

```cpp
#pragma once
#include "graph.hpp"
#include "pr_plan.hpp"

#ifdef SS_PR_WAVETIME
#include <cstdio>
#include <cstdlib>
#include <string>
#endif

namespace {

constexpr int MAXK = 16;

struct PrCtl {
    double S[MAXK];
    double delta[MAXK];
    double csum[MAXK];
    double xz[MAXK];
    double xz_in[MAXK];
    double tele[MAXK];
    int32_t active[MAXK];
    int32_t iters[MAXK];
    int32_t sweep;
    int32_t n_active;
    uint32_t ticket;
    uint32_t stuck;
    uint32_t gticket[8];
};

constexpr int AFF_MAXK = 256;
constexpr unsigned AFF_NB = 512;
struct AffCtl {
    double u[AFF_MAXK];
    double delta[AFF_MAXK];
    int32_t active[AFF_MAXK], iters[AFF_MAXK], just[AFF_MAXK];
    double r_x, r_prev, r_next;
    double s_x, s_prev, s_next;
    double xz_prev[2];
    int32_t n_active, n_just, k_real, it;
};

struct PrParams {
    const uint32_t* in_ptr;
    const uint32_t* in_src;
    const uint32_t* outdeg;
    double* x;
    const double* tab_rd[2];
    double* tab_wr[2];
    const WorkItem* work;
    double* partials;
    double* segpart;
    uint32_t* rowticket;
    PrCtl* ctl;
    const double* x0;
    double d, teleport, eps, tele_n;
    int32_t max_iter, k_topics, world;
    uint32_t sl_nd, cnt_nd, sl_d, cnt_d, seg_edges, n_items;
    uint32_t pos_nd, pos_d;
    const uint32_t* memb;
    const double* tin;
    const double* nz_in;
    uint32_t ts_mask;
    uint32_t zrow;
    const uint32_t* woff;
    uint32_t stagger_div;
    uint32_t stagger_code;
    uint32_t class_order;
    uint32_t n_order;
    double* x_alt;
    AffCtl* aff;
    const double* tele_col;
    const uint32_t* sh_deg;
    uint32_t n_shared;
    uint32_t share;
    uint32_t tab_rows;
};

}

enum PrKernel : int {
    PR_STEP = 0,
    PR_SWEEP = 1,
    PR_SWEEP_N = 2,
};

struct ss_pr {
    ss_graph* g = nullptr;
    PrKernel kernel = PR_SWEEP;
    int gw = 1;
    ss::DevBuf<float> wire_send, wire_recv;
    bool nwave = false;
    int persist_mode = 1;
    bool persist = false;
    int k = 1;
    PrParams prm{};
    unsigned nblocks = 0;
    ss::DevBuf<double> x, tab0, tab1, send, partials, segpart, x0;
    ss::DevBuf<uint32_t> rowticket;
    ss::DevBuf<uint32_t> memb;
    ss::DevBuf<double> tin, nz_in;
    ss::DevBuf<WorkItem> work;
    ss::DevBuf<uint32_t> woff;
    ss::DevBuf<uint32_t> src_shared;
    ss::DevBuf<uint32_t> sh_deg;
    ss::DevBuf<PrCtl> ctl;
    bool begun = false;
    bool need_finalize = false;
    bool finalize_is_begin = false;
};

#pragma GCC visibility push(hidden)
namespace ss {
unsigned begin_blocks(const ss_pr* pr);
void pr_launch_begin(ss_pr* pr, hipStream_t st, unsigned nb);
void pr_launch_step(ss_pr* pr, hipStream_t st);
void pr_launch_finalize(ss_pr* pr, hipStream_t st, int is_begin);
void pr_sweep_launch(ss_pr* pr, hipStream_t st);
int pr_sweep_occupancy(int gw);
void pr_sweep_n_launch(ss_pr* pr, hipStream_t st);
int pr_sweep_n_occupancy(int gw);
void pr_multi_n_launch(ss_pr* pr, hipStream_t st, int n_steps);
int pr_multi_n_occupancy(int gw);
void pr_step_launch(ss_pr* pr, hipStream_t st);
int pr_step_occupancy(int gw);
#ifdef SS_PR_WAVETIME
void pr_dump_wave_times(const ss_pr* pr);
#endif
size_t pr_wire_floats(const ss_pr* pr);
hipError_t pr_wire_alloc(ss_pr* pr);
void pr_wire_pack(ss_pr* pr, hipStream_t st);
void pr_wire_unpack(ss_pr* pr, hipStream_t st);
}
#pragma GCC visibility pop

namespace {
#ifdef SS_PR_WAVETIME
inline FILE* open_dump(const char* name) {
    const char* dir = getenv("SS_PR_WAVETIME_DIR");
    return fopen((std::string(dir && *dir ? dir : ".") + "/" + name).c_str(), "w");
}
#endif
inline int32_t read_ctl(ss_ctx* ctx, const ss_pr* pr, hipStream_t st, const char* what, const PrCtl** out) {
    ctx->pin_used = 0;
    PrCtl* const hp = ctx->pin<PrCtl>();
    if (hipMemcpyAsync(hp, pr->ctl.p, sizeof(PrCtl), hipMemcpyDeviceToHost, st) != hipSuccess) return ctx->fail(SS_ERR_HIP, "%s: status read failed", what);
    SS_TRY(ss::sync_bounded(ctx, st, what));
    *out = hp;
    return SS_OK;
}
}
```

spaghettisearch_amd/csrc/pr_sweep.hip:

```cpp
#include "pr_device.hpp"

#include <algorithm>

namespace {

template <int GW>
__device__ __forceinline__ double tab_at(const double* __restrict__ T, uint32_t row, int t) {
    return *reinterpret_cast<const double*>(reinterpret_cast<const char*>(T) + (size_t)((row * (uint32_t)GW + (uint32_t)t) * 8u));
}


template <int GW, bool TS>
struct SweepCtx {
    const PrParams& p;
    const double* __restrict__ T;
    double* __restrict__ Tw;
    double S, x0;
    bool act;
    int t, gbase, slot;
    double dsum, csum;
};

__device__ __forceinline__ uint32_t turn_fill(uint32_t epos, uint32_t lim) {
    return min((uint32_t)CH, __builtin_elementwise_sub_sat(lim, epos));
}

template <int GW>
__device__ __forceinline__ void idx_turn(const uint32_t* __restrict__ in_src, uint32_t epos, uint32_t n, uint32_t zrow, int t, uint32_t (&src)[CH / GW]) {
#pragma unroll
    for (int r = 0; r < CH / GW; r++) {
        const uint32_t j = (uint32_t)(r * GW + t);
        const uint32_t raw = NT_LOAD(&in_src[j < n ? epos + j : 0u]);
        src[r] = j < n ? (raw & SRC_MASK) : zrow;
    }
}
template <int GW>
__device__ __forceinline__ void gather_turn(const double* __restrict__ T, const uint32_t (&src)[CH / GW], int t, int gbase, double (&v)[CH]) {
#pragma unroll
    for (int j = 0; j < CH; j++) {
        const uint32_t sj = (uint32_t)__shfl((int)src[j / GW], gbase + (j % GW), 64);
        v[j] = tab_at<GW>(T, sj, t);
    }
}

template <int GW, bool TS>
__device__ __forceinline__ void finish_row(SweepCtx<GW, TS>& c, uint32_t lrow, double y, double xo, uint32_t od) {
    const PrParams& p = c.p;
    y += c.x0;
    const size_t xi = (size_t)lrow * GW + c.t;
    double tele = p.teleport;
    if constexpr (TS) tele = teleport_of(p, lrow, c.t);
    double xn = (y + tele) / c.S;
    if (c.act) {
        NT_STORE(xn, &p.x[xi]);
        c.dsum += fabs(xn - xo);
    } else {
        xn = xo;
    }
    if (lrow < p.sl_nd) {
        const double cc = p.d * xn / (double)od;
        NT_STORE(cc, &c.Tw[xi]);
        c.csum += cc;
    }
}

template <int GW, bool TS>
__device__ __forceinline__ void long_rows(SweepCtx<GW, TS>& c, const WorkItem* __restrict__ work, uint32_t i0, uint32_t i1, int lane) {
    constexpr int NS = 64 / GW;
    constexpr uint32_t TW = NS * CH;
    const PrParams& p = c.p;
    if (i0 >= i1) return;
    WorkItem cur = work[i0], nxt = work[i0 + 1];
    uint32_t src_n[CH / GW];
    {
        const uint32_t e0 = cur.beg + (uint32_t)c.slot * CH;
        idx_turn<GW>(p.in_src, e0, turn_fill(e0, cur.end), p.zrow, c.t, src_n);
    }
    for (uint32_t it = i0; it < i1; it++) {
        const WorkItem nn = work[it + 2];
        const uint32_t lrow = cur.row;
        const double xo = NT_LOAD(&p.x[(size_t)lrow * GW + c.t]);
        const uint32_t od = lrow < p.sl_nd ? NT_LOAD(&p.outdeg[lrow]) : 1u;
        const uint32_t turns = (cur.end - cur.beg + TW - 1) / TW;
        const bool more = it + 1 < i1;
        double acc = 0.0;
        for (uint32_t i = 0; i < turns; i++) {
            uint32_t src[CH / GW];
#pragma unroll
            for (int r = 0; r < CH / GW; r++) src[r] = src_n[r];
            const bool last = i + 1 == turns;
            const uint32_t e1 = (last ? nxt.beg : cur.beg + (i + 1) * TW) + (uint32_t)c.slot * CH;
            const uint32_t lim = last ? (more ? nxt.end : 0u) : cur.end;
            idx_turn<GW>(p.in_src, e1, turn_fill(e1, lim), p.zrow, c.t, src_n);
            double v[CH];
            gather_turn<GW>(c.T, src, c.t, c.gbase, v);
#pragma unroll
            for (int j = 0; j < CH; j++) acc += v[j];
        }
        const double y = wave_sum_topic<GW>(acc);
        if (cur.kind == V_ROWW) {
            if (lane < GW) finish_row<GW>(c, lrow, y, xo, od);
        } else {
            if (lane < GW) __hip_atomic_store(&p.segpart[(size_t)(cur.sbase + cur.count) * GW + c.t], y, __ATOMIC_RELAXED, __HIP_MEMORY_SCOPE_AGENT);
            asm volatile("s_waitcnt vmcnt(0)" ::: "memory");
            unsigned prev = 0;
            if (lane == 0) prev = __hip_atomic_fetch_add(&p.rowticket[cur.tix], 1u, __ATOMIC_RELAXED, __HIP_MEMORY_SCOPE_AGENT);
            prev = (unsigned)__builtin_amdgcn_readfirstlane((int)prev);
            if (prev == cur.nseg - 1) {
                if (lane == 0) __hip_atomic_store(&p.rowticket[cur.tix], 0u, __ATOMIC_RELAXED, __HIP_MEMORY_SCOPE_AGENT);
                if (lane < GW) {
                    double ys = 0.0;
                    for (uint32_t q = 0; q < cur.nseg; q++)
                        ys += __hip_atomic_load(&p.segpart[(size_t)(cur.sbase + q) * GW + c.t], __ATOMIC_RELAXED, __HIP_MEMORY_SCOPE_AGENT);
                    finish_row<GW>(c, lrow, ys, xo, od);
                }
            }
        }
        cur = nxt;
        nxt = nn;
    }
}

template <int GW, bool TS>
__device__ __forceinline__ void quad_rows(SweepCtx<GW, TS>& c, const WorkItem* __restrict__ work, uint32_t i0, uint32_t i1) {
    constexpr int NS = 64 / GW;
    const PrParams& p = c.p;
    if (i0 >= i1) return;
    const uint32_t myq = (uint32_t)c.t * NS + (uint32_t)c.slot;
    auto bounds = [&](const WorkItem& w, bool live, uint32_t& bv, uint32_t& ev, uint32_t& ov) __attribute__((always_inline)) {
        const bool have = live && myq < w.count;
        const uint32_t rq = live ? w.row + (have ? myq : 0u) : 0u;
        const uint32_t b = p.in_ptr[rq], e = p.in_ptr[rq + 1];
        bv = b;
        ev = have ? e : b;
        ov = rq < p.sl_nd ? NT_LOAD(&p.outdeg[rq]) : 1u;
    };
    WorkItem cur = work[i0], nxt = work[i0 + 1];
    uint32_t cb, ce, co, nb, ne, no;
    bounds(cur, true, cb, ce, co);
    bounds(nxt, i0 + 1 < i1, nb, ne, no);
    uint32_t it = i0, q = 0, ch = 0;
    uint32_t nq = (cur.count + NS - 1) / NS, nch = cur.nseg;
    uint32_t src_n[CH / GW];
    {
        const uint32_t b0 = (uint32_t)__shfl((int)cb, c.gbase, 64), e0 = (uint32_t)__shfl((int)ce, c.gbase, 64);
        idx_turn<GW>(p.in_src, b0, turn_fill(b0, e0), p.zrow, c.t, src_n);
    }
    double acc = 0.0;
    while (it < i1) {
        uint32_t src[CH / GW];
#pragma unroll
        for (int r = 0; r < CH / GW; r++) src[r] = src_n[r];
        uint32_t qn = q, cn = ch + 1;
        bool cross = false;
        if (cn == nch) {
            cn = 0;
            qn = q + 1;
            if (qn == nq) { qn = 0; cross = true; }
        }
        const bool live_n = !cross || it + 1 < i1;
        {
            const uint32_t b_n = (uint32_t)__shfl((int)(cross ? nb : cb), c.gbase + (int)qn, 64);
            const uint32_t e_n = (uint32_t)__shfl((int)(cross ? ne : ce), c.gbase + (int)qn, 64);
            const uint32_t ep = b_n + cn * CH;
            idx_turn<GW>(p.in_src, ep, live_n ? turn_fill(ep, e_n) : 0u, p.zrow, c.t, src_n);
        }
        const bool ends = ch + 1 == nch;
        const uint32_t lrow = cur.row + q * NS + (uint32_t)c.slot;
        const bool valid = q * NS + (uint32_t)c.slot < cur.count;
        double xo = 0.0;
        if (ends) xo = NT_LOAD(&p.x[(size_t)(valid ? lrow : cur.row) * GW + c.t]);
        double v[CH];
        gather_turn<GW>(c.T, src, c.t, c.gbase, v);
#pragma unroll
        for (int j = 0; j < CH; j++) acc += v[j];
        if (ends) {
            const uint32_t od = (uint32_t)__shfl((int)co, c.gbase + (int)q, 64);
            if (valid) finish_row<GW>(c, lrow, acc, xo, od);
            acc = 0.0;
        }
        q = qn;
        ch = cn;
        if (cross) {
            it++;
            cur = nxt;
            cb = nb; ce = ne; co = no;
            nq = (cur.count + NS - 1) / NS;
            nch = cur.nseg;
            nxt = work[it + 1];
            bounds(nxt, it + 1 < i1, nb, ne, no);
        }
    }
}

template <int GW, int R, bool TS>
__device__ __forceinline__ void deg_rows(SweepCtx<GW, TS>& c, const WorkItem* __restrict__ work, uint32_t i0, uint32_t i1) {
    constexpr int NS = 64 / GW;
    constexpr int DM = CH / R;
    constexpr int IR = CH / GW;
    const PrParams& p = c.p;
    if (i0 >= i1) return;
    auto idx = [&](const WorkItem& w, bool live, uint32_t turn, uint32_t (&src)[IR]) __attribute__((always_inline)) {
        const uint32_t rb = (turn * NS + (uint32_t)c.slot) * R;
#pragma unroll
        for (int r = 0; r < IR; r++) {
            const uint32_t j = (uint32_t)(r * GW + c.t);
            const uint32_t rr = rb + j / DM, u = j % DM;
            const bool ok = live && u < w.nseg && rr < w.count;
            const uint32_t raw = NT_LOAD(&p.in_src[ok ? w.beg + rr * w.nseg + u : 0u]);
            src[r] = ok ? (raw & SRC_MASK) : p.zrow;
        }
    };
    WorkItem cur = work[i0], nxt = work[i0 + 1];
    uint32_t src_n[IR];
    idx(cur, true, 0, src_n);
    for (uint32_t it = i0; it < i1; it++) {
        const WorkItem nn = work[it + 2];
        const uint32_t row0 = cur.row, count = cur.count;
        const uint32_t turns = (count + NS * R - 1) / (NS * R);
        for (uint32_t i = 0; i < turns; i++) {
            uint32_t src[IR];
#pragma unroll
            for (int r = 0; r < IR; r++) src[r] = src_n[r];
            if (i + 1 < turns) idx(cur, true, i + 1, src_n);
            else idx(nxt, it + 1 < i1, 0, src_n);
            const uint32_t rb = (i * NS + (uint32_t)c.slot) * R;
            double xo[R];
#pragma unroll
            for (int r = 0; r < R; r++) xo[r] = NT_LOAD(&p.x[(size_t)(row0 + (rb + r < count ? rb + r : 0u)) * GW + c.t]);
            const uint32_t myr = row0 + (rb + (uint32_t)c.t < count ? rb + (uint32_t)c.t : 0u);
            const uint32_t odv = (c.t < R && myr < p.sl_nd) ? NT_LOAD(&p.outdeg[myr]) : 1u;
            double v[CH];
            gather_turn<GW>(c.T, src, c.t, c.gbase, v);
#pragma unroll
            for (int r = 0; r < R; r++) {
                double y = 0.0;
#pragma unroll
                for (int u = 0; u < DM; u++) y += v[r * DM + u];
                const uint32_t od = (uint32_t)__shfl((int)odv, c.gbase + r, 64);
                if (rb + r < count) finish_row<GW>(c, row0 + rb + r, y, xo[r], od);
            }
        }
        cur = nxt;
        nxt = nn;
    }
}

#ifndef SS_PR_MINW
#define SS_PR_MINW 1
#endif
#ifdef SS_PR_WAVETIME
__device__ unsigned long long g_pr_wt[65536][2];
#endif
template <int GW, bool TS>
__global__ __launch_bounds__(TPB, SS_PR_MINW) void k_pr_sweep(PrParams p) {
    constexpr int NS = 64 / GW;
    PrCtl* ctl = p.ctl;
    if (ctl->n_active == 0) return;
#ifdef SS_PR_WAVETIME
    unsigned long long wt0;
    asm volatile("s_memrealtime %0\n\ts_waitcnt lgkmcnt(0)" : "=s"(wt0));
#endif
    const int sweep = ctl->sweep;
    const int lane = threadIdx.x & 63;
    const uint32_t wave = (uint32_t)__builtin_amdgcn_readfirstlane((int)(threadIdx.x >> 6));
    SweepCtx<GW, TS> c{p, p.tab_rd[sweep & 1], p.tab_wr[sweep & 1], 0.0, 0.0, false, lane % GW, lane - lane % GW, lane / GW, 0.0, 0.0};
    c.S = ctl->S[c.t];
    c.act = ctl->active[c.t] != 0;
    c.x0 = sweep == 0 ? p.x0[c.t] : 0.0;

    if constexpr (!TS) {
        if (p.n_shared) {
            const double xz_out = c.act ? zero_row_rank(p, sweep, c.S, p.x0[c.t]) : ctl->xz[c.t];
            const uint32_t nel = p.n_shared * (uint32_t)GW;
            for (uint32_t i = blockIdx.x * TPB + threadIdx.x; i < nel; i += gridDim.x * TPB)
                c.Tw[(size_t)(p.zrow + 1) * GW + i] = p.d * xz_out / (double)p.sh_deg[i / GW];
        }
    }

    const uint32_t* __restrict__ off = p.woff + (size_t)(blockIdx.x * WAVES + wave) * 8;
    int rot = p.stagger_div ? (int)((blockIdx.x / p.stagger_div) % 6u) : 0;
    if (p.stagger_code) {
        uint32_t cdv = p.stagger_code;
        for (uint32_t r = blockIdx.x / p.stagger_div; r > 0; r--) cdv /= 6u;
        rot = (int)(cdv % 6u);
    }
    for (int s6 = 0; s6 < 6; s6++) {
    const int cls = (int)((p.class_order >> (3 * ((s6 + rot) % 6))) & 7u);
    {
        int ln = lane;
        asm volatile("" : "+v"(ln));
        c.t = ln % GW;
        c.gbase = ln - ln % GW;
        c.slot = ln / GW;
    }
    switch (cls) {
    case 0: long_rows<GW>(c, p.work, off[0], off[1], lane); break;
    case 1: quad_rows<GW>(c, p.work, off[1], off[2]); break;
    case 2: deg_rows<GW, 2>(c, p.work, off[2], off[3]); break;
    case 3: deg_rows<GW, 4>(c, p.work, off[3], off[4]); break;
    case 4: deg_rows<GW, 8>(c, p.work, off[4], off[5]); break;
    default:
    for (uint32_t item = off[5]; item < off[6]; item++) {
        const WorkItem w = p.work[item];
        const bool store = TS || !p.share;
        const bool ts = TS && p.memb && ((p.ts_mask >> c.t) & 1u);
        const double xz_out = c.act ? (ts ? zero_row_rank_ts(p, sweep, c.S, p.x0[c.t], 0.0) : zero_row_rank(p, sweep, c.S, p.x0[c.t])) : ctl->xz[c.t];
        const double xz_inn = ts ? (c.act ? zero_row_rank_ts(p, sweep, c.S, p.x0[c.t], p.tin[c.t]) : ctl->xz_in[c.t]) : xz_out;
        uint32_t od[16];
#pragma unroll
        for (int i = 0; i < 16; i++) {
            const uint32_t rr = (uint32_t)(i * NS + c.slot);
            od[i] = NT_LOAD(&p.outdeg[w.row + (rr < w.count ? rr : 0u)]);
        }
#pragma unroll
        for (int i = 0; i < 16; i++) {
            const uint32_t rr = (uint32_t)(i * NS + c.slot);
            if (rr < w.count) {
                const uint32_t lrow = w.row + rr;
                const double xz = ts && ((p.memb[lrow] >> c.t) & 1u) ? xz_inn : xz_out;
                const double cc = p.d * xz / (double)od[i];
                if (store) NT_STORE(cc, &c.Tw[(size_t)lrow * GW + c.t]);
                c.csum += cc;
            }
        }
    }
    break;
    }
    }
#ifdef SS_PR_WAVETIME
    {
        unsigned long long wt1;
        asm volatile("s_waitcnt vmcnt(0)\n\ts_memrealtime %0\n\ts_waitcnt lgkmcnt(0)" : "=s"(wt1));
        const uint32_t wid = (blockIdx.x * WAVES + wave) & 65535u;
        if (lane == 0) { g_pr_wt[wid][0] = wt0; g_pr_wt[wid][1] = wt1; }
    }
#endif
    block_reduce_and_publish<GW>(p, c.dsum, c.csum, c.Tw, false);
}

template __device__ void begin_caller_context<8, 16>(const PrParams&, double*);

}

namespace ss {
void pr_sweep_launch(ss_pr* pr, hipStream_t st) {
    const bool ts = pr->prm.memb != nullptr;
    if (pr->gw == 8) {
        if (ts) hipLaunchKernelGGL((k_pr_sweep<8, true>), dim3(pr->nblocks), dim3(TPB), 0, st, pr->prm);
        else hipLaunchKernelGGL((k_pr_sweep<8, false>), dim3(pr->nblocks), dim3(TPB), 0, st, pr->prm);
    } else {
        if (ts) hipLaunchKernelGGL((k_pr_sweep<16, true>), dim3(pr->nblocks), dim3(TPB), 0, st, pr->prm);
        else hipLaunchKernelGGL((k_pr_sweep<16, false>), dim3(pr->nblocks), dim3(TPB), 0, st, pr->prm);
    }
}
int pr_sweep_occupancy(int gw) {
    int per_cu = 8;
    if (gw == 8) (void)hipOccupancyMaxActiveBlocksPerMultiprocessor(&per_cu, k_pr_sweep<8, false>, TPB, 0);
    else (void)hipOccupancyMaxActiveBlocksPerMultiprocessor(&per_cu, k_pr_sweep<16, false>, TPB, 0);
    return per_cu;
}

#ifdef SS_PR_WAVETIME
void pr_dump_wave_times(const ss_pr* pr) {
    if (pr->gw < 8) return;
    (void)hipDeviceSynchronize();
    const uint32_t nwv = std::min<uint32_t>(65536u, pr->nblocks * WAVES);
    std::vector<unsigned long long> h((size_t)nwv * 2);
    if (hipMemcpyFromSymbol(h.data(), HIP_SYMBOL(g_pr_wt), h.size() * sizeof(unsigned long long)) != hipSuccess || !nwv) return;
    unsigned long long t0 = ~0ull;
    for (uint32_t w = 0; w < nwv; w++) t0 = std::min(t0, h[2 * w]);
    std::vector<double> st(nwv), en(nwv);
    for (uint32_t w = 0; w < nwv; w++) { st[w] = (double)(h[2 * w] - t0) / 100.0; en[w] = (double)(h[2 * w + 1] - t0) / 100.0; }
    std::sort(st.begin(), st.end()); std::sort(en.begin(), en.end());
    if (FILE* f = open_dump("pr_wt.csv")) {
        fprintf(f, "wave,start_us,end_us\n");
        for (uint32_t w = 0; w < nwv; w++) fprintf(f, "%u,%.2f,%.2f\n", w, (double)(h[2 * w] - t0) / 100.0, (double)(h[2 * w + 1] - t0) / 100.0);
        fclose(f);
    }
    fprintf(stderr, "[pr wavetime] %u waves: start us median %.1f max %.1f | out of items us min %.1f p10 %.1f median %.1f p90 %.1f p99 %.1f max %.1f\n", nwv,
            st[nwv / 2], st[nwv - 1], en[0], en[nwv / 10], en[nwv / 2], en[nwv * 9 / 10], en[(size_t)nwv * 99 / 100], en[nwv - 1]);
}
#endif
}
```

Measured before the change: 18640.

## Add opt-in twin-rank sharing for one-in-edge rows in PageRank sweep

Adds an optional plan that groups rows with exactly one in-edge by their source. Each group's rank is computed once per bundle and fanned out to the member rows' contribution table, using a new work-item class, device buffers and host-side planning. Rank readback and teardown (untwin) are changed to match. The path is gated behind a new option that defaults off. Separately, the default SS_PR_MINW launch bound changes from 1 to 4, which affects every sweep and trades registers for occupancy.

New measurement: 18250. 2.1% lower.

```diff
diff --git a/spaghettisearch_amd/csrc/ctx.hip b/spaghettisearch_amd/csrc/ctx.hip
--- a/spaghettisearch_amd/csrc/ctx.hip
+++ b/spaghettisearch_amd/csrc/ctx.hip
@@ -280,6 +280,7 @@
     "pr.stagger",
     "pr.deal_global",
     "pr.share_zero_rows",
+    "pr.share_twin_ranks",
     "pr.item_turns",
     "graph.late_free",
     "pr.trace",
diff --git a/spaghettisearch_amd/csrc/pagerank.hip b/spaghettisearch_amd/csrc/pagerank.hip
--- a/spaghettisearch_amd/csrc/pagerank.hip
+++ b/spaghettisearch_amd/csrc/pagerank.hip
@@ -47,6 +47,17 @@
     }
 }
 
+__global__ __launch_bounds__(TPB) void k_pr_twin_fetch(const uint32_t* __restrict__ in_ptr, const uint32_t* __restrict__ in_src, const uint32_t* __restrict__ outdeg,
+                                                       uint32_t one_nd, uint32_t n1_nd, uint32_t row_d, uint32_t n1, uint32_t* __restrict__ src_out,
+                                                       uint32_t* __restrict__ od_out) {
+    const uint32_t i = blockIdx.x * TPB + threadIdx.x;
+    if (i >= n1) return;
+    const bool nd = i < n1_nd;
+    const uint32_t row = nd ? one_nd + i : row_d + (i - n1_nd);
+    src_out[i] = in_src[in_ptr[row]] & SRC_MASK;
+    od_out[i] = nd ? outdeg[row] : 0u;
+}
+
 template <int GW>
 __global__ __launch_bounds__(TPB) void k_pr_begin(PrParams p) {
     const int lane = threadIdx.x & 63;
@@ -56,6 +67,8 @@
     double csum = 0.0;
     for (uint32_t i = blockIdx.x * TPB + threadIdx.x; i < p.n_shared * (uint32_t)GW; i += gridDim.x * TPB)
         Tw[(size_t)(p.zrow + 1) * GW + i] = p.d * x0 / (double)p.sh_deg[i / GW];
+    if (p.twin)
+        for (size_t i = (size_t)blockIdx.x * TPB + threadIdx.x; i < (size_t)p.tw_rows * GW; i += (size_t)gridDim.x * TPB) p.tw_x[i] = x0;
     const size_t n_el = ((size_t)p.sl_nd + p.sl_d) * GW;
     for (size_t i = (size_t)blockIdx.x * TPB + threadIdx.x; i < n_el; i += (size_t)gridDim.x * TPB) {
         const uint32_t lrow = (uint32_t)(i / GW);
@@ -88,11 +101,20 @@
 }
 
 template <int GW>
+__device__ __forceinline__ const double* twin_rank_row(const TwinRead& tw, const double* x, uint32_t lrow, uint32_t sl_nd, bool zero) {
+    if (tw.slot && !zero) {
+        if (lrow < sl_nd) { if (lrow >= tw.one_nd) return tw.x + (size_t)tw.slot[lrow - tw.one_nd] * GW; }
+        else if (lrow - sl_nd >= tw.one_d) return tw.x + (size_t)tw.slot[tw.n1_nd + (lrow - sl_nd - tw.one_d)] * GW;
+    }
+    return x + (size_t)lrow * GW;
+}
+
+template <int GW>
 __global__ void k_pr_read(const double* __restrict__ x, const PrCtl* __restrict__ ctl, const uint32_t* __restrict__ old_id,
                           uint32_t sl_nd, uint32_t cnt_nd, uint32_t pos_nd, uint32_t sl_d, uint32_t cnt_d, uint32_t pos_d,
                           uint64_t id0_nd, uint64_t id0_d, int k_topics, uint64_t out_stride,
                           int by_original_id, uint32_t* __restrict__ ids_out, double* __restrict__ out,
-                          const uint32_t* __restrict__ memb, uint32_t ts_mask) {
+                          const uint32_t* __restrict__ memb, uint32_t ts_mask, TwinRead tw) {
     const size_t n_rows = (size_t)cnt_nd + cnt_d;
     size_t i = (size_t)blockIdx.x * blockDim.x + threadIdx.x;
     if (i >= n_rows) return;
@@ -103,8 +125,9 @@
     if (ids_out) ids_out[i] = orig;
     const bool zero = lrow < sl_nd ? lrow >= pos_nd : (lrow - sl_nd) >= pos_d;
     const uint32_t mb = memb ? memb[lrow] & ts_mask : 0u;
+    const double* const xrow = twin_rank_row<GW>(tw, x, lrow, sl_nd, zero);
     for (int k = 0; k < k_topics; k++)
-        out[(size_t)k * out_stride + o] = zero ? (((mb >> k) & 1u) ? ctl->xz_in[k] : ctl->xz[k]) : x[(size_t)lrow * GW + k];
+        out[(size_t)k * out_stride + o] = zero ? (((mb >> k) & 1u) ? ctl->xz_in[k] : ctl->xz[k]) : xrow[k];
 }
 
 __global__ void k_pr_memb(const uint64_t* __restrict__ set_ptr, const uint32_t* __restrict__ set_nodes, int k_topics, uint64_t n_nodes,
@@ -218,19 +241,20 @@
 template <int GW>
 __global__ __launch_bounds__(TPB) void k_pr_read_orig(const double* __restrict__ x, const PrCtl* __restrict__ ctl, const uint32_t* __restrict__ new_id,
                                                       uint64_t n, uint32_t sl_nd, uint32_t pos_nd, uint32_t pos_d, int k_topics,
-                                                      double* __restrict__ out, const uint32_t* __restrict__ memb, uint32_t ts_mask) {
+                                                      double* __restrict__ out, const uint32_t* __restrict__ memb, uint32_t ts_mask, TwinRead tw) {
     const uint64_t v = (uint64_t)blockIdx.x * blockDim.x + threadIdx.x;
     if (v >= n) return;
     const uint32_t lrow = new_id[v];
     const bool zero = lrow < sl_nd ? lrow >= pos_nd : (lrow - sl_nd) >= pos_d;
     double r[GW];
     if (!zero) {
+        const double* const xrow = twin_rank_row<GW>(tw, x, lrow, sl_nd, false);
         if constexpr (GW >= 2) {
-            const double2* const row = reinterpret_cast<const double2*>(x + (size_t)lrow * GW);
+            const double2* const row = reinterpret_cast<const double2*>(xrow);
 #pragma unroll
             for (int j = 0; j < GW / 2; j++) { const double2 t = row[j]; r[2 * j] = t.x; r[2 * j + 1] = t.y; }
         } else {
-            r[0] = x[lrow];
+            r[0] = xrow[0];
         }
     } else {
         const uint32_t mb = memb ? memb[lrow] & ts_mask : 0u;
@@ -249,14 +273,14 @@
     if (!n_rows) return;
     if (by_orig && g->world == 1 && !ids && stride == g->n) {
         hipLaunchKernelGGL(k_pr_read_orig<GW>, dim3(ss::div_up(g->n, TPB)), dim3(TPB), 0, st, (const double*)pr->x.p, (const PrCtl*)pr->ctl.p,
-                           (const uint32_t*)g->new_id.p, g->n, g->sl_nd, pr->prm.pos_nd, pr->prm.pos_d, pr->k, out, pr->prm.memb, pr->prm.ts_mask);
+                           (const uint32_t*)g->new_id.p, g->n, g->sl_nd, pr->prm.pos_nd, pr->prm.pos_d, pr->k, out, pr->prm.memb, pr->prm.ts_mask, pr->tw_read);
         return;
     }
     hipLaunchKernelGGL(k_pr_read<GW>, dim3(ss::div_up(n_rows, TPB)), dim3(TPB), 0, st, (const double*)pr->x.p,
                        (const PrCtl*)pr->ctl.p, (const uint32_t*)g->old_id.p, g->sl_nd, g->cnt_nd, pr->prm.pos_nd, g->sl_d, g->cnt_d,
                        pr->prm.pos_d,
                        (uint64_t)g->rank * g->sl_nd, g->nd_int + (uint64_t)g->rank * g->sl_d, pr->k, stride, by_orig, ids, out,
-                       pr->prm.memb, pr->prm.ts_mask);
+                       pr->prm.memb, pr->prm.ts_mask, pr->tw_read);
 }
 
 #define SS_GW_DISPATCH(gw, fn, ...)          \
@@ -367,7 +391,7 @@
     p.woff = pr->woff.p;
     p.stagger_div = opt.stagger != 0 ? (uint32_t)std::max(g->ctx->cu_count, 1) : 0u;
     p.stagger_code = opt.stagger >= 10 ? (uint32_t)(opt.stagger - 10) : 0u;
-    p.class_order = pack_class_order(opt.class_order);
+    p.class_order = opt.twin ? pack_class_order7(opt.class_order) : pack_class_order(opt.class_order);
     p.n_order = pack_n_order(opt.n_class_order);
 }
 
@@ -402,6 +426,79 @@
     }
     return SS_OK;
 }
+#ifdef SS_PR_WAVETIME
+void dump_wave_loads(const Cut& cut, const std::vector<double>& cost, const std::vector<uint32_t>& owner, uint32_t nw);
+#endif
+const std::vector<uint32_t>& deal_plan(const ss_ctx* ctx, ss_pr* pr, Cut& cut, const PlanOptions& opt, int gi, bool trace) {
+    static const std::vector<uint32_t> no_woff;
+    const ss_graph* g = pr->g;
+    auto t_now = [] { return std::chrono::steady_clock::now(); };
+    auto t_ms = [](std::chrono::steady_clock::time_point a, std::chrono::steady_clock::time_point b) { return std::chrono::duration<double, std::milli>(b - a).count(); };
+    const auto tc1 = t_now();
+    const int per_cu = blocks_per_cu(pr->kernel, pr->gw);
+    const auto tc1a = t_now();
+    pr->nblocks = grid_for(ctx, pr, opt, per_cu, cut.items.size());
+    if (pr->kernel == PR_STEP) return no_woff;
+    const uint32_t nw = pr->nblocks * WAVES;
+    const auto td0 = t_now();
+    const std::vector<double>& cost = item_costs(cut, g->h_indeg_nd, g->h_indeg_d, g->sl_nd, gi, pr->nwave);
+    const auto td0a = t_now();
+    std::vector<uint32_t>& owner = deal_items(cut, cost, nw, pr->nwave, opt);
+#ifdef SS_PR_WAVETIME
+    dump_wave_loads(cut, cost, owner, nw);
+#endif
+    const auto td1 = t_now();
+    if (trace) fprintf(stderr, "[pr trace]   deal: occupancy query %.2f ms, costs %.3f ms, owners %.3f ms\n", t_ms(tc1, tc1a), t_ms(td0, td0a), t_ms(td0a, td1));
+    const std::vector<uint32_t>& woff = place_items(cut, owner, nw);
+    if (trace) fprintf(stderr, "[pr trace]   deal: placement %.3f ms\n", t_ms(td1, t_now()));
+    return woff;
+}
+int32_t upload_plan(ss_pr* pr, const Cut& cut, const std::vector<uint32_t>& woff, hipStream_t st) {
+    const ss_graph* g = pr->g;
+    ss_ctx* ctx = g->ctx;
+    const size_t GW = (size_t)pr->gw;
+    const std::vector<WorkItem>& items = cut.items;
+    SS_HIP(ctx, pr->partials.alloc(((size_t)std::max(pr->nblocks, ss::begin_blocks(pr)) + 8) * 2 * GW));
+    SS_HIP(ctx, pr->segpart.alloc((size_t)std::max(cut.nsegs, 1u) * GW));
+    SS_HIP(ctx, pr->rowticket.alloc(std::max(cut.nmulti, 1u)));
+    SS_HIP(ctx, hipMemsetAsync(pr->rowticket.p, 0, pr->rowticket.bytes(), st));
+    SS_HIP(ctx, pr->woff.alloc(std::max<size_t>(woff.size(), 8)));
+    if (!woff.empty()) SS_HIP(ctx, hipMemcpyAsync(pr->woff.p, woff.data(), woff.size() * sizeof(uint32_t), hipMemcpyHostToDevice, st));
+    SS_HIP(ctx, pr->work.alloc(items.size()));
+    SS_HIP(ctx, hipMemcpyAsync(pr->work.p, items.data(), items.size() * sizeof(WorkItem), hipMemcpyHostToDevice, st));
+    if (pr->kernel != PR_STEP)
+        hipLaunchKernelGGL(k_pr_item_ranges, dim3(ss::div_up(items.size(), TPB)), dim3(TPB), 0, st, pr->work.p, (uint32_t)items.size(), (const uint32_t*)g->in_ptr.p);
+    return SS_OK;
+}
+int32_t untwin_ranks(ss_pr* pr, hipStream_t st) {
+    if (!pr->prm.twin) return SS_OK;
+    ss_graph* g = pr->g;
+    ss_ctx* ctx = g->ctx;
+    SS_HIP(ctx, hipStreamSynchronize(st));
+    const PlanOptions opt = plan_options(ctx, pr, g->n_local());
+    Cut cut = cut_items(g->h_indeg_nd, g->h_indeg_d, g->sl_nd, pr->gw, pr->nwave, opt);
+    const std::vector<uint32_t>& woff = deal_plan(ctx, pr, cut, opt, pr->gw, false);
+    SS_TRY(upload_plan(pr, cut, woff, st));
+    SS_HIP(ctx, hipStreamSynchronize(st));
+    for (auto* b : {&pr->tw_src, &pr->tw_od, &pr->tw_row, &pr->tw_slot}) b->release();
+    pr->tw_x.release();
+    pr->tw_read = TwinRead{};
+    PrParams& p = pr->prm;
+    p.work = pr->work.p;
+    p.woff = pr->woff.p;
+    p.partials = pr->partials.p;
+    p.segpart = pr->segpart.p;
+    p.rowticket = pr->rowticket.p;
+    p.seg_edges = cut.seg_edges;
+    p.n_items = (uint32_t)cut.items.size();
+    p.class_order = pack_class_order(opt.class_order);
+    p.tw_src = p.tw_od = p.tw_row = nullptr;
+    p.tw_x = nullptr;
+    p.tw_rows = 0;
+    p.twin = 0;
+    return SS_OK;
+}
+
 int32_t unshare_rows(ss_pr* pr, hipStream_t st) {
     if (!pr->prm.share) return SS_OK;
     const ss_graph* g = pr->g;
@@ -459,7 +556,6 @@
     pr->k = k_topics;
     pick_kernel(ctx, pr, k_topics, g->nd_int);
     const int GW = pr->gw;
-    const bool vitems = pr->kernel != PR_STEP;
     const int GI = pr->nwave ? 8 : GW;
     const size_t n_local = g->n_local();
     if (((uint64_t)g->nd_int + 1) * GW * 8 >= (1ull << 32))
@@ -474,48 +570,70 @@
     if (!share) SS_TRY(alloc_tables(pr, st, (size_t)g->nd_int + 1));
 
     const auto tc0 = t_now();
-    const PlanOptions opt = plan_options(ctx, pr, n_local);
+    bool twin = GW >= 8 && g->world == 1 && ctx->opt("pr.affine", 0) == 0 && ctx->opt("pr.share_twin_ranks", 0) != 0;
+    PlanOptions opt = plan_options(ctx, pr, n_local);
+    opt.twin = twin;
     Cut cut = cut_items(g->h_indeg_nd, g->h_indeg_d, g->sl_nd, GI, pr->nwave, opt);
+    const uint32_t n1_nd = cut.pos_nd - cut.one_nd, n1 = n1_nd + (cut.pos_d - cut.one_d);
+    if (twin && n1 == 0) twin = opt.twin = false;
     const uint32_t n_tail = g->cnt_nd - cut.pos_nd;
     struct PinGuard { ss_ctx* c; void* p = nullptr; size_t cap = 0; ~PinGuard() { c->pin_free(p, cap); } } tail_od{ctx};
     if (share && n_tail == 0) {
         share = false;
         SS_TRY(alloc_tables(pr, st, (size_t)g->nd_int + 1));
     }
-    if (share) {
+    PinGuard twin_in{ctx};
+    ss::DevBuf<uint32_t> d_twin_in;
+    if ((share || twin) && n_tail) {
         tail_od.p = ctx->pin_alloc((size_t)n_tail * sizeof(uint32_t), &tail_od.cap);
         if (!tail_od.p) return ctx->fail(SS_ERR_OOM, "ss_pr_create: no pinned host memory for %u out-degrees", n_tail);
         SS_HIP(ctx, hipMemcpyAsync(tail_od.p, g->outdeg.p + cut.pos_nd, (size_t)n_tail * sizeof(uint32_t), hipMemcpyDeviceToHost, st));
     }
     const auto tc1 = t_now();
-    const int per_cu = blocks_per_cu(pr->kernel, GW);
-    const auto tc1a = t_now();
-    pr->nblocks = grid_for(ctx, pr, opt, per_cu, cut.items.size());
-    static const std::vector<uint32_t> no_woff;
-    const std::vector<uint32_t>* woff = &no_woff;
-    if (vitems) {
-        const uint32_t nw = pr->nblocks * WAVES;
-        const auto td0 = t_now();
-        const std::vector<double>& cost = item_costs(cut, g->h_indeg_nd, g->h_indeg_d, g->sl_nd, GI, pr->nwave);
-        const auto td0a = t_now();
-        std::vector<uint32_t>& owner = deal_items(cut, cost, nw, pr->nwave, opt);
-#ifdef SS_PR_WAVETIME
-        dump_wave_loads(cut, cost, owner, nw);
-#endif
-        const auto td1 = t_now();
-        if (trace) fprintf(stderr, "[pr trace]   deal: occupancy query %.2f ms, costs %.3f ms, owners %.3f ms\n", t_ms(tc1, tc1a), t_ms(td0, td0a), t_ms(td0a, td1));
-        woff = &place_items(cut, owner, nw);
-        if (trace) fprintf(stderr, "[pr trace]   deal: placement %.3f ms\n", t_ms(td1, t_now()));
-    }
+    SharedRows sh;
+    bool have_sh = false;
+    TwinPlan tp;
+    if (twin) {
+        SS_HIP(ctx, d_twin_in.alloc((size_t)n1 * 2));
+        twin_in.p = ctx->pin_alloc((size_t)n1 * 2 * sizeof(uint32_t), &twin_in.cap);
+        if (!twin_in.p) return ctx->fail(SS_ERR_OOM, "ss_pr_create: no pinned host memory for %u one-in-edge rows", n1);
+        hipLaunchKernelGGL(k_pr_twin_fetch, dim3(ss::div_up((size_t)n1, TPB)), dim3(TPB), 0, st, (const uint32_t*)g->in_ptr.p, (const uint32_t*)g->in_src.p,
+                           (const uint32_t*)g->outdeg.p, cut.one_nd, n1_nd, g->sl_nd + cut.one_d, n1, d_twin_in.p, d_twin_in.p + n1);
+        SS_HIP(ctx, hipMemcpyAsync(twin_in.p, d_twin_in.p, (size_t)n1 * 2 * sizeof(uint32_t), hipMemcpyDeviceToHost, st));
+        SS_HIP(ctx, hipStreamSynchronize(st));
+        const auto tt0 = t_now();
+        if (n_tail) { sh = plan_shared_rows(static_cast<const uint32_t*>(tail_od.p), n_tail, cut.pos_nd); have_sh = true; }
+        uint32_t* const h_src = static_cast<uint32_t*>(twin_in.p);
+        const uint32_t* const h_od = h_src + n1;
+        std::vector<uint32_t> key(n1);
+        for (uint32_t i = 0; i < n1; i++) {
+            const uint32_t sv = h_src[i];
+            key[i] = sv < cut.pos_nd || !have_sh ? sv : sh.row_of(static_cast<const uint32_t*>(tail_od.p)[std::min(sv - cut.pos_nd, n_tail - 1)]);
+            if (share) h_src[i] = key[i];
+        }
+        if (!plan_twin_ranks(key.data(), h_src, h_od, n1, n1_nd, cut.one_nd, tp))
+            return ctx->fail(SS_ERR_UNSUPPORTED, "ss_pr_create: %u one-in-edge rows do not fit the twin plan", n1);
+        if ((uint64_t)tp.rank_rows() * GW * 8 >= (1ull << 32)) {
+            twin = opt.twin = false;
+            tp = TwinPlan();
+            const Cut again = cut_items(g->h_indeg_nd, g->h_indeg_d, g->sl_nd, GI, pr->nwave, opt);
+            cut.nsegs = again.nsegs; cut.nmulti = again.nmulti; cut.seg_edges = again.seg_edges;
+            cut.pos_nd = again.pos_nd; cut.pos_d = again.pos_d; cut.one_nd = again.one_nd; cut.one_d = again.one_d;
+            std::copy(again.vbeg, again.vbeg + 8, cut.vbeg);
+        } else {
+            add_twin_items(cut, tp, GI, opt);
+        }
+        if (trace) fprintf(stderr, "[pr trace]   twin ranks: %u one-in-edge rows -> %zu groups in %u bundles (host %.3f ms)\n", n1, tp.groups.size(), tp.n_bundles, t_ms(tt0, t_now()));
+    }
+    const std::vector<uint32_t>* woff = &deal_plan(ctx, pr, cut, opt, GI, trace);
     const std::vector<WorkItem>& items = cut.items;
 
     g->settle();
     const auto tc2 = t_now();
-    SharedRows sh;
     if (share) {
         SS_HIP(ctx, hipStreamSynchronize(st));
         const auto ts0 = t_now();
-        sh = plan_shared_rows(static_cast<const uint32_t*>(tail_od.p), n_tail, cut.pos_nd);
+        if (!have_sh) sh = plan_shared_rows(static_cast<const uint32_t*>(tail_od.p), n_tail, cut.pos_nd);
         const auto ts1 = t_now();
         SS_TRY(alloc_tables(pr, st, (size_t)sh.table_rows));
         SS_HIP(ctx, pr->sh_deg.alloc(sh.deg.size()));
@@ -528,16 +646,18 @@
         if (trace) fprintf(stderr, "[pr trace]   shared rows: %u rows without in-edges -> %zu shared rows (host %.3f ms), table %llu rows\n", n_tail, sh.deg.size(),
                            t_ms(ts0, ts1), (unsigned long long)sh.table_rows);
     }
-    SS_HIP(ctx, pr->partials.alloc(((size_t)std::max(pr->nblocks, ss::begin_blocks(pr)) + 8) * 2 * GW));
-    SS_HIP(ctx, pr->segpart.alloc((size_t)std::max(cut.nsegs, 1u) * GW));
-    SS_HIP(ctx, pr->rowticket.alloc(std::max(cut.nmulti, 1u)));
-    SS_HIP(ctx, hipMemsetAsync(pr->rowticket.p, 0, pr->rowticket.bytes(), st));
-    SS_HIP(ctx, pr->woff.alloc(std::max<size_t>(woff->size(), 8)));
-    if (!woff->empty()) SS_HIP(ctx, hipMemcpyAsync(pr->woff.p, woff->data(), woff->size() * sizeof(uint32_t), hipMemcpyHostToDevice, st));
-    SS_HIP(ctx, pr->work.alloc(items.size()));
-    SS_HIP(ctx, hipMemcpyAsync(pr->work.p, items.data(), items.size() * sizeof(WorkItem), hipMemcpyHostToDevice, st));
-    if (vitems)
-        hipLaunchKernelGGL(k_pr_item_ranges, dim3(ss::div_up(items.size(), TPB)), dim3(TPB), 0, st, pr->work.p, (uint32_t)items.size(), (const uint32_t*)g->in_ptr.p);
+    SS_TRY(upload_plan(pr, cut, *woff, st));
+    if (twin) {
+        SS_HIP(ctx, pr->tw_src.alloc(tp.b_src.size()));
+        SS_HIP(ctx, pr->tw_od.alloc(tp.b_od.size()));
+        SS_HIP(ctx, pr->tw_row.alloc(tp.b_row.size()));
+        SS_HIP(ctx, pr->tw_slot.alloc(tp.slot.size()));
+        SS_HIP(ctx, pr->tw_x.alloc((size_t)tp.rank_rows() * GW));
+        SS_HIP(ctx, hipMemcpyAsync(pr->tw_src.p, tp.b_src.data(), tp.b_src.size() * sizeof(uint32_t), hipMemcpyHostToDevice, st));
+        SS_HIP(ctx, hipMemcpyAsync(pr->tw_od.p, tp.b_od.data(), tp.b_od.size() * sizeof(uint32_t), hipMemcpyHostToDevice, st));
+        SS_HIP(ctx, hipMemcpyAsync(pr->tw_row.p, tp.b_row.data(), tp.b_row.size() * sizeof(uint32_t), hipMemcpyHostToDevice, st));
+        SS_HIP(ctx, hipMemcpyAsync(pr->tw_slot.p, tp.slot.data(), tp.slot.size() * sizeof(uint32_t), hipMemcpyHostToDevice, st));
+    }
     SS_HIP(ctx, pr->ctl.alloc(1));
     SS_HIP(ctx, hipMemsetAsync(pr->ctl.p, 0, sizeof(PrCtl), st));
     double h_x0[MAXK];
@@ -559,6 +679,16 @@
         p.zrow = sh.zrow;
         p.tab_rows = cut.pos_nd;
     }
+    if (twin) {
+        PrParams& p = pr->prm;
+        p.tw_src = pr->tw_src.p;
+        p.tw_od = pr->tw_od.p;
+        p.tw_row = pr->tw_row.p;
+        p.tw_x = pr->tw_x.p;
+        p.tw_rows = tp.rank_rows();
+        p.twin = 1;
+        pr->tw_read = TwinRead{pr->tw_slot.p, pr->tw_x.p, cut.one_nd, cut.one_d, n1_nd};
+    }
     if (trace) trace_plan(pr, items, *woff);
     g->users++;
     *out = guard.release();
@@ -580,6 +710,7 @@
     const ss_graph* g = pr->g;
     const int K = pr->k;
     SS_TRY(unshare_rows(pr, st));
+    SS_TRY(untwin_ranks(pr, st));
     std::vector<uint64_t> h_ptr(K + 1);
     SS_HIP(ctx, ss::copy_in(ctx->stream, h_ptr.data(), set_ptr, (K + 1) * sizeof(uint64_t)));
     if (h_ptr[0] != 0) return ctx->fail(SS_ERR_INVALID, "ss_pr_set_teleport: set_ptr[0] != 0");
diff --git a/spaghettisearch_amd/csrc/pr_plan.hpp b/spaghettisearch_amd/csrc/pr_plan.hpp
--- a/spaghettisearch_amd/csrc/pr_plan.hpp
+++ b/spaghettisearch_amd/csrc/pr_plan.hpp
@@ -18,7 +18,8 @@
                   V_ROWW = 9,
                   V_QUAD = 10,
                   V_DEG = 11,
-                  V_ZERO = 12 };
+                  V_ZERO = 12,
+                  V_TWIN = 13 };
 
 struct WorkItem {
     uint32_t kind;
@@ -43,6 +44,7 @@
     int64_t class_order = 235401;
     int64_t n_class_order = 2310;
     int64_t stagger = 0;
+    bool twin = false;
 };
 
 struct PlanScratch {
@@ -63,7 +65,8 @@
     uint32_t nsegs = 0, nmulti = 0;
     uint32_t seg_edges = 0;
     uint32_t pos_nd = 0, pos_d = 0;
-    uint32_t vbeg[7] = {0};
+    uint32_t one_nd = 0, one_d = 0;
+    uint32_t vbeg[8] = {0};
 };
 
 inline Cut cut_items(const ss::SortedDegrees& nd, const ss::SortedDegrees& d, uint32_t sl_nd, int gw, bool lane_rows, const PlanOptions& opt) {
@@ -79,7 +82,7 @@
     auto &vseg = s.vseg, &vroww = s.vroww, &vquad = s.vquad, &vzero = s.vzero;
     auto& vdeg = s.vdeg;
     for (auto* v : {&seg, &rwg, &wav, &grp, &zer, &vseg, &vroww, &vquad, &vdeg[0], &vdeg[1], &vdeg[2], &vzero}) v->clear();
-    auto emit_v = [&](const ss::SortedDegrees& deg, uint32_t row0, bool non_dangling, uint32_t& n_pos) {
+    auto emit_v = [&](const ss::SortedDegrees& deg, uint32_t row0, bool non_dangling, uint32_t& n_pos, uint32_t& n_one) {
         const uint32_t cnt = (uint32_t)deg.size();
         const uint32_t T_MULTI = 4096, T_DEG = 8;
         const uint32_t T_QUAD = opt.t_quad;
@@ -115,9 +118,14 @@
             vquad.push_back({V_QUAD, row0 + r, rows, nch, 0, 0});
             r += rows;
         }
+        n_one = UINT32_MAX;
         while (r < cnt && deg_at(r) > 0) {
             const uint32_t D = deg_at(r);
             const uint32_t run = deg.start[j_at + 1] - r;
+            if (D == 1) {
+                n_one = r;
+                if (opt.twin) { r += run; continue; }
+            }
             const uint32_t R = D <= 2 ? 8 : D <= 4 ? 4 : 2;
             const uint32_t per_item = lane_rows ? 64u * item_turns : NSLOT * R * item_turns;
             auto& out = vdeg[R == 2 ? 0 : R == 4 ? 1 : 2];
@@ -125,12 +133,13 @@
             r += run;
         }
         n_pos = r;
+        if (n_one == UINT32_MAX) n_one = r;
         const uint32_t ZERO_ROWS = 16 * NSLOT;
         if (non_dangling)
             for (uint32_t o = r; o < cnt; o += ZERO_ROWS) vzero.push_back({V_ZERO, row0 + o, std::min<uint32_t>(ZERO_ROWS, cnt - o), 0, 0, 0});
     };
-    auto emit = [&](const ss::SortedDegrees& deg, uint32_t row0, bool non_dangling, uint32_t& n_pos) {
-        if (gw >= 8) { emit_v(deg, row0, non_dangling, n_pos); return; }
+    auto emit = [&](const ss::SortedDegrees& deg, uint32_t row0, bool non_dangling, uint32_t& n_pos, uint32_t& n_one) {
+        if (gw >= 8) { emit_v(deg, row0, non_dangling, n_pos, n_one); return; }
         const uint32_t cnt = (uint32_t)deg.size();
         const uint32_t a = deg.first_at_most(T_SEG);
         const uint32_t c = std::max(a, deg.first_at_most(0));
@@ -146,14 +155,14 @@
             const uint32_t GROUP_ROWS = WAVES * NSLOT * 4;
             for (uint32_t r = b; r < c; r += GROUP_ROWS) grp.push_back({W_GROUP, row0 + r, std::min<uint32_t>(GROUP_ROWS, c - r), 0, 0, 0});
         }
-        n_pos = c;
+        n_pos = n_one = c;
         const uint32_t ZERO_ROWS = (TPB * 8) / gw;
         if (non_dangling)
             for (uint32_t r = c; r < cnt; r += ZERO_ROWS) zer.push_back({W_ZERO, row0 + r, std::min<uint32_t>(ZERO_ROWS, cnt - r), 0, 0, 0});
     };
-    emit(nd, 0, true, cut.pos_nd);
+    emit(nd, 0, true, cut.pos_nd, cut.one_nd);
     const size_t vquad_split = vquad.size();
-    emit(d, sl_nd, false, cut.pos_d);
+    emit(d, sl_nd, false, cut.pos_d, cut.one_d);
     auto& items = cut.items;
     auto& vbeg = cut.vbeg;
     items.clear();
@@ -176,8 +185,8 @@
     }
     vbeg[5] = (uint32_t)items.size();
     items.insert(items.end(), vzero.begin(), vzero.end());
-    vbeg[6] = (uint32_t)items.size();
     if (items.empty()) items.push_back({W_ZERO, 0, 0, 0, 0, 0});
+    vbeg[6] = vbeg[7] = (uint32_t)items.size();
     return cut;
 }
 
@@ -210,6 +219,7 @@
                 turns = (double)plan_div_up(w.count, NS * R) * (R == 8 ? 2.5 : R == 4 ? 1.7 : 1.3);
                 break;
             }
+            case V_TWIN: turns = (double)plan_div_up(w.count, NS) * 2.5; break;
             default: turns = 0.5; break;
         }
         cost[i] = turns + 1.0;
@@ -236,8 +246,8 @@
         bucket.assign(NB + 1, 0u);
         order.resize(n_items);
         size_t c0 = 0;
-        for (int kcls = 0; kcls < (deal_mode == 2 ? 6 : 1); kcls++) {
-            const size_t c1 = deal_mode == 2 ? (kcls < 5 ? std::min<size_t>(cut.vbeg[kcls + 1], n_items) : n_items) : n_items;
+        for (int kcls = 0; kcls < (deal_mode == 2 ? 7 : 1); kcls++) {
+            const size_t c1 = deal_mode == 2 ? (kcls < 6 ? std::min<size_t>(cut.vbeg[kcls + 1], n_items) : n_items) : n_items;
             if (kcls) std::fill(bucket.begin(), bucket.end(), 0u);
             for (size_t i = c0; i < c1; i++) bucket[bkey(i) + 1]++;
             for (uint32_t b = 0; b < NB; b++) bucket[b + 1] += bucket[b];
@@ -281,8 +291,8 @@
     auto &woff = s.woff, &cnt = s.cnt;
     woff.assign((size_t)nw * 8, 0);
     cnt.assign((size_t)nw * 8, 0);
-    for (int k = 0; k < 6; k++) {
-        const size_t i1 = k < 5 ? std::min<size_t>(cut.vbeg[k + 1], items.size()) : items.size();
+    for (int k = 0; k < 7; k++) {
+        const size_t i1 = k < 6 ? std::min<size_t>(cut.vbeg[k + 1], items.size()) : items.size();
         for (size_t i = std::min<size_t>(cut.vbeg[k], i1); i < i1; i++) { owner[i] = owner[i] * 8 + (uint32_t)k; cnt[owner[i]]++; }
     }
     uint32_t run_off = 0;
@@ -310,6 +320,25 @@
         if (c < 6) seen |= 1u << c;
     }
     return seen == 0x3Fu ? packed : (0u | 1u << 3 | 2u << 6 | 3u << 9 | 4u << 12 | 5u << 15);
+}
+inline uint32_t pack_class_order7(int64_t code) {
+    uint32_t packed = 0, seen = 0;
+    int64_t c7 = code;
+    for (int pos = 6; pos >= 0; pos--) {
+        const uint32_t c = (uint32_t)(c7 % 10);
+        c7 /= 10;
+        packed |= (c & 7u) << (3 * pos);
+        if (c < 7) seen |= 1u << c;
+    }
+    if (seen == 0x7Fu && c7 == 0) return packed;
+    const uint32_t six = pack_class_order(code);
+    packed = 0;
+    for (int pos = 0, out = 0; pos < 6; pos++) {
+        const uint32_t c = (six >> (3 * pos)) & 7u;
+        packed |= c << (3 * out++);
+        if (c == 2) packed |= 6u << (3 * out++);
+    }
+    return packed;
 }
 inline uint32_t pack_n_order(int64_t code) {
     uint32_t packed = 0, seen = 0;
@@ -352,4 +381,79 @@
     return sh;
 }
 
-}
+constexpr uint32_t TWIN_HEADS = 8, TWIN_SLOTS = 16, TWIN_PIECE = 16;
+constexpr uint32_t TWIN_NONE = 0xFFFFFFFFu;
+constexpr uint32_t TWIN_ROW_MASK = 0x03FFFFFFu;
+constexpr uint32_t TWIN_HEAD_SHIFT = 26;
+constexpr uint32_t TWIN_VALID = 0x80000000u;
+struct TwinGroup {
+    uint32_t src, first, count;
+};
+struct TwinPlan {
+    std::vector<TwinGroup> groups;
+    std::vector<uint32_t> od;
+    std::vector<uint32_t> trow;
+    std::vector<uint32_t> slot;
+    std::vector<uint32_t> b_src, b_od, b_row;
+    uint32_t n_bundles = 0;
+    uint32_t rank_rows() const { return n_bundles * TWIN_HEADS; }
+};
+inline bool plan_twin_ranks(const uint32_t* key, const uint32_t* src, const uint32_t* od, size_t n1, size_t n1_nd, uint32_t one_nd, TwinPlan& tp) {
+    tp = TwinPlan();
+    if (!n1) return true;
+    if ((uint64_t)one_nd + n1_nd > (uint64_t)TWIN_ROW_MASK + 1 || n1 > (size_t)1 << 31) return false;
+    std::vector<uint64_t> a(n1), b(n1);
+    uint32_t hi = 0;
+    for (size_t i = 0; i < n1; i++) { a[i] = (uint64_t)key[i] << 32 | (uint64_t)i; hi = std::max(hi, key[i]); }
+    for (int shift = 0; shift < 32 && (hi >> shift) != 0; shift += 11) {
+        size_t cnt[2049] = {0};
+        for (size_t i = 0; i < n1; i++) cnt[((a[i] >> (32 + shift)) & 2047u) + 1]++;
+        for (int q = 0; q < 2048; q++) cnt[q + 1] += cnt[q];
+        for (size_t i = 0; i < n1; i++) b[cnt[(a[i] >> (32 + shift)) & 2047u]++] = a[i];
+        a.swap(b);
+    }
+    tp.od.resize(n1);
+    tp.trow.resize(n1);
+    tp.slot.resize(n1);
+    auto open_bundle = [&] {
+        tp.n_bundles++;
+        tp.b_src.resize((size_t)tp.n_bundles * TWIN_HEADS, TWIN_NONE);
+        tp.b_od.resize((size_t)tp.n_bundles * TWIN_SLOTS, 0u);
+        tp.b_row.resize((size_t)tp.n_bundles * TWIN_SLOTS, 0u);
+    };
+    tp.b_src.reserve(n1 + TWIN_HEADS);
+    tp.b_od.reserve(2 * n1 + TWIN_SLOTS);
+    tp.b_row.reserve(2 * n1 + TWIN_SLOTS);
+    uint32_t heads = TWIN_HEADS, used = TWIN_SLOTS;
+    for (size_t m = 0; m < n1;) {
+        size_t e = m + 1;
+        while (e < n1 && e - m < TWIN_PIECE && (a[e] >> 32) == (a[m] >> 32)) e++;
+        const uint32_t count = (uint32_t)(e - m);
+        if (heads == TWIN_HEADS || used + count > TWIN_SLOTS) { open_bundle(); heads = 0; used = 0; }
+        const uint32_t bun = tp.n_bundles - 1;
+        const uint32_t first_ix = (uint32_t)(a[m] & 0xFFFFFFFFu);
+        tp.groups.push_back({src[first_ix], (uint32_t)m, count});
+        tp.b_src[(size_t)bun * TWIN_HEADS + heads] = src[first_ix];
+        for (size_t q = m; q < e; q++, used++) {
+            const uint32_t ix = (uint32_t)(a[q] & 0xFFFFFFFFu);
+            const bool nd = ix < n1_nd;
+            tp.od[q] = nd ? od[ix] : 0u;
+            tp.trow[q] = nd ? one_nd + ix : TWIN_NONE;
+            tp.slot[ix] = bun * TWIN_HEADS + heads;
+            tp.b_od[(size_t)bun * TWIN_SLOTS + used] = tp.od[q];
+            tp.b_row[(size_t)bun * TWIN_SLOTS + used] = TWIN_VALID | heads << TWIN_HEAD_SHIFT | (nd ? one_nd + ix : 0u);
+        }
+        heads++;
+        m = e;
+    }
+    return true;
+}
+inline void add_twin_items(Cut& cut, const TwinPlan& tp, int gw, const PlanOptions& opt) {
+    const uint32_t per_item = (uint32_t)(64 / gw) * opt.item_turns;
+    cut.vbeg[6] = (uint32_t)cut.items.size();
+    for (uint32_t b = 0; b < tp.n_bundles; b += per_item)
+        cut.items.push_back({V_TWIN, b, std::min(per_item, tp.n_bundles - b), 0, 0, 0, 0, 0});
+    cut.vbeg[7] = (uint32_t)cut.items.size();
+}
+
+}
diff --git a/spaghettisearch_amd/csrc/pr_state.hpp b/spaghettisearch_amd/csrc/pr_state.hpp
--- a/spaghettisearch_amd/csrc/pr_state.hpp
+++ b/spaghettisearch_amd/csrc/pr_state.hpp
@@ -74,6 +74,18 @@
     uint32_t n_shared;
     uint32_t share;
     uint32_t tab_rows;
+    const uint32_t* tw_src;
+    const uint32_t* tw_od;
+    const uint32_t* tw_row;
+    double* tw_x;
+    uint32_t tw_rows;
+    uint32_t twin;
+};
+
+struct TwinRead {
+    const uint32_t* slot;
+    const double* x;
+    uint32_t one_nd, one_d, n1_nd;
 };
 
 }
@@ -103,6 +115,9 @@
     ss::DevBuf<uint32_t> woff;
     ss::DevBuf<uint32_t> src_shared;
     ss::DevBuf<uint32_t> sh_deg;
+    ss::DevBuf<uint32_t> tw_src, tw_od, tw_row, tw_slot;
+    ss::DevBuf<double> tw_x;
+    TwinRead tw_read{};
     ss::DevBuf<PrCtl> ctl;
     bool begun = false;
     bool need_finalize = false;
diff --git a/spaghettisearch_amd/csrc/pr_sweep.hip b/spaghettisearch_amd/csrc/pr_sweep.hip
--- a/spaghettisearch_amd/csrc/pr_sweep.hip
+++ b/spaghettisearch_amd/csrc/pr_sweep.hip
@@ -246,8 +246,97 @@
     }
 }
 
+__device__ __forceinline__ double pick8(double a0, double a1, double a2, double a3, double a4, double a5, double a6, double a7, uint32_t h) {
+    const double b0 = (h & 1u) ? a1 : a0, b1 = (h & 1u) ? a3 : a2, b2 = (h & 1u) ? a5 : a4, b3 = (h & 1u) ? a7 : a6;
+    const double c0 = (h & 2u) ? b1 : b0, c1 = (h & 2u) ? b3 : b2;
+    return (h & 4u) ? c1 : c0;
+}
+template <int GW>
+__device__ __forceinline__ double* twin_x_at(double* __restrict__ X, uint32_t row, int t) {
+    return reinterpret_cast<double*>(reinterpret_cast<char*>(X) + (size_t)((row * (uint32_t)GW + (uint32_t)t) * 8u));
+}
+template <int GW>
+__device__ __forceinline__ void twin_rows(SweepCtx<GW, false>& c, const WorkItem* __restrict__ work, uint32_t i0, uint32_t i1) {
+    constexpr int NS = 64 / GW;
+    constexpr int IR = (int)TWIN_SLOTS / GW;
+    static_assert(TWIN_HEADS == 8 && TWIN_SLOTS == CH && GW >= (int)TWIN_HEADS, "a lane group's turn: 8 heads, 16 member slots");
+    const PrParams& p = c.p;
+    if (i0 >= i1) return;
+    struct Words { uint32_t hs, mo[IR], mr[IR]; };
+    auto idx = [&](const WorkItem& w, bool live, uint32_t turn, Words& x) __attribute__((always_inline)) {
+        const uint32_t bi = turn * NS + (uint32_t)c.slot;
+        const bool ok = live && bi < w.count;
+        const uint32_t b = ok ? w.row + bi : 0u;
+        const uint32_t hs = NT_LOAD(&p.tw_src[(size_t)b * TWIN_HEADS + ((uint32_t)c.t & (TWIN_HEADS - 1))]);
+        x.hs = ok ? hs : TWIN_NONE;
+#pragma unroll
+        for (int r = 0; r < IR; r++) {
+            const size_t j = (size_t)b * TWIN_SLOTS + (uint32_t)(r * GW + c.t);
+            x.mo[r] = NT_LOAD(&p.tw_od[j]);
+            const uint32_t mr = NT_LOAD(&p.tw_row[j]);
+            x.mr[r] = ok ? mr : 0u;
+        }
+    };
+    WorkItem cur = work[i0], nxt = work[i0 + 1];
+    Words wn;
+    idx(cur, true, 0, wn);
+    for (uint32_t it = i0; it < i1; it++) {
+        const WorkItem nn = work[it + 2];
+        const uint32_t b0 = cur.row, count = cur.count;
+        const uint32_t turns = (count + NS - 1) / NS;
+        for (uint32_t i = 0; i < turns; i++) {
+            const Words w = wn;
+            if (i + 1 < turns) idx(cur, true, i + 1, wn);
+            else idx(nxt, it + 1 < i1, 0, wn);
+            const uint32_t bi = i * NS + (uint32_t)c.slot;
+            const uint32_t xr0 = (b0 + (bi < count ? bi : 0u)) * TWIN_HEADS;
+            double xo[TWIN_HEADS], v[TWIN_HEADS];
+            bool live[TWIN_HEADS];
+#pragma unroll
+            for (int r = 0; r < (int)TWIN_HEADS; r++) {
+                const uint32_t sr = (uint32_t)__shfl((int)w.hs, c.gbase + r, 64);
+                live[r] = sr != TWIN_NONE;
+                xo[r] = NT_LOAD(twin_x_at<GW>(p.tw_x, xr0 + (live[r] ? (uint32_t)r : 0u), c.t));
+                v[r] = tab_at<GW>(c.T, live[r] ? sr : p.zrow, c.t);
+            }
+            double xn[TWIN_HEADS], dv[TWIN_HEADS];
+#pragma unroll
+            for (int r = 0; r < (int)TWIN_HEADS; r++) {
+                double y = 0.0;
+                y += v[r];
+                y += c.x0;
+                xn[r] = (y + p.teleport) / c.S;
+                if (c.act) {
+                    if (live[r]) NT_STORE(xn[r], twin_x_at<GW>(p.tw_x, xr0 + (uint32_t)r, c.t));
+                    dv[r] = fabs(xn[r] - xo[r]);
+                } else {
+                    xn[r] = xo[r];
+                    dv[r] = 0.0;
+                }
+            }
+#pragma unroll
+            for (int j = 0; j < (int)TWIN_SLOTS; j++) {
+                const uint32_t mr = (uint32_t)__shfl((int)w.mr[j / GW], c.gbase + (j % GW), 64);
+                const uint32_t od = (uint32_t)__shfl((int)w.mo[j / GW], c.gbase + (j % GW), 64);
+                const uint32_t h = (mr >> TWIN_HEAD_SHIFT) & (TWIN_HEADS - 1);
+                const bool real = (mr & TWIN_VALID) != 0;
+                const double xs = pick8(xn[0], xn[1], xn[2], xn[3], xn[4], xn[5], xn[6], xn[7], h);
+                const double ds = pick8(dv[0], dv[1], dv[2], dv[3], dv[4], dv[5], dv[6], dv[7], h);
+                c.dsum += real ? ds : 0.0;
+                if (real && od != 0) {
+                    const double cc = p.d * xs / (double)od;
+                    NT_STORE(cc, &c.Tw[(size_t)(mr & TWIN_ROW_MASK) * GW + c.t]);
+                    c.csum += cc;
+                }
+            }
+        }
+        cur = nxt;
+        nxt = nn;
+    }
+}
+
 #ifndef SS_PR_MINW
-#define SS_PR_MINW 1
+#define SS_PR_MINW 4
 #endif
 #ifdef SS_PR_WAVETIME
 __device__ unsigned long long g_pr_wt[65536][2];
@@ -279,14 +368,15 @@
     }
 
     const uint32_t* __restrict__ off = p.woff + (size_t)(blockIdx.x * WAVES + wave) * 8;
+    const int ncls = !TS && p.twin ? 7 : 6;
     int rot = p.stagger_div ? (int)((blockIdx.x / p.stagger_div) % 6u) : 0;
     if (p.stagger_code) {
         uint32_t cdv = p.stagger_code;
         for (uint32_t r = blockIdx.x / p.stagger_div; r > 0; r--) cdv /= 6u;
         rot = (int)(cdv % 6u);
     }
-    for (int s6 = 0; s6 < 6; s6++) {
-    const int cls = (int)((p.class_order >> (3 * ((s6 + rot) % 6))) & 7u);
+    for (int s6 = 0; s6 < ncls; s6++) {
+    const int cls = (int)((p.class_order >> (3 * ((s6 + rot) % ncls))) & 7u);
     {
         int ln = lane;
         asm volatile("" : "+v"(ln));
@@ -300,6 +390,9 @@
     case 2: deg_rows<GW, 2>(c, p.work, off[2], off[3]); break;
     case 3: deg_rows<GW, 4>(c, p.work, off[3], off[4]); break;
     case 4: deg_rows<GW, 8>(c, p.work, off[4], off[5]); break;
+    case 6:
+        if constexpr (!TS) twin_rows<GW>(c, p.work, off[6], off[7]);
+        break;
     default:
     for (uint32_t item = off[5]; item < off[6]; item++) {
         const WorkItem w = p.work[item];
```
